# 0kam/alproj

Measured on AMD Instinct MI355X. Metric: Gpoints/s projected (pinhole + Brown-Conrady, single pose) over the 100M-vertex DSM; CMA-ES iterations/s in `cma`, higher is better.
Workload: dtype f32

## Files before the change

### alproj_amd/csrc/alp_raster.hip

```cpp
#include "alp_raster_internal.h"

#include <algorithm>
#include <atomic>
#include <climits>
#include <cmath>
#include <cstdlib>
#include <thread>
#include <type_traits>
#include <vector>

namespace alp {

#include "raster_dev.h"
#include "raster_common.h"
#include "raster_parked.h"
#include "raster_index.h"
#include "raster_plan.h"
#include "raster_grid.h"
#include "raster_large.h"
#include "raster_resolve.h"
#include "raster_post.h"

}

// ... 97 lines not shown
    for (auto &s : sums) {
        const unsigned here = s;
        s = (unsigned)run;
        run += here;
    }
    if ((long long)run != m->n_tri) return ALP_OK;
    e = hipMemcpyAsync(block_dev, sums.data(), (size_t)blocks * 4, hipMemcpyHostToDevice, st);
    if (e == hipSuccess) {
        hipLaunchKernelGGL(subgrid_rank_kernel, dim3((unsigned)blocks), dim3(256), 0, st, present, words, block_dev, rank);
        e = hipStreamSynchronize(st);
    }
    if (e != hipSuccess) return fail(ALP_EHIP, "sub-grid ranks: %s", hipGetErrorString(e));
    block_dev.reset();
    m->valid_derived = std::move(derived);
    if (int rc = apply_derived_mask(m, nullptr)) {
        reset_all(m->valid_derived, m->valid);
        return rc;
    }
    m->tri_present = std::move(present);
    m->tri_rank = std::move(rank);
    m->ind.reset();
    m->implicit = true;
    m->grid_h = gh;
    m->grid_w = gw;
    m->n_tri = full;
    return ALP_OK;
}

int ensure_gqueue(alp_mesh *m, unsigned cap) {
    if (m->gqueue && m->gcap >= cap) return ALP_OK;
    m->gcap = 0;
    if (int rc = m->gqueue.reserve((size_t)cap * sizeof(unsigned))) return rc;
    m->gcap = cap;
    return ALP_OK;
}

int finish_frame_of(alp_mesh *m);

int frame_valid_count(alp_mesh *m, int64_t *count) {
    if (int e = finish_frame_of(m)) return e;
    const long long npix = (long long)m->w * m->h;
    const int chunks = (int)((npix + COMPACT_CHUNK - 1) / COMPACT_CHUNK);
    if (chunks > m->compact_cap) {
        m->compact_cap = 0;
        reset_all(m->compact_counts, m->compact_offsets);
        const size_t counts = (size_t)chunks * (sizeof(unsigned) + 4 * sizeof(float)) + 16;
        const size_t offsets = (size_t)(chunks + 3) * sizeof(unsigned long long);
        if (int rc = reserve_all({counts, offsets}, m->compact_counts, m->compact_offsets)) return rc;
        m->compact_cap = chunks;
    }
    hipStream_t st = ctx().stream;
    ktime_begin();
    float *span = (float *)(((uintptr_t)(m->compact_counts + chunks) + 15) & ~(uintptr_t)15);
    hipLaunchKernelGGL(valid_count_kernel, dim3(chunks), dim3(256), 0, st, m->image, npix, m->compact_counts, span);
    hipLaunchKernelGGL(scan_counts_kernel, dim3(1), dim3(1024), 0, st, m->compact_counts, chunks, m->compact_offsets, span);
    ktime_end();
    ALP_HIP(hipGetLastError());
    unsigned long long tail[3] = {0, 0, 0};
    ALP_HIP(hipMemcpyAsync(tail, m->compact_offsets + chunks, sizeof(tail), hipMemcpyDeviceToHost, st));
    ALP_HIP(hipStreamSynchronize(st));
    const unsigned long long total = tail[0];
    memcpy(m->valid_span, tail + 1, sizeof(m->valid_span));
    m->valid_total = (int64_t)total;
    *count = m->valid_total;
    return ALP_OK;
}

int frame_valid_write(alp_mesh *m, const double *offsets, unsigned *idx_dev, double *xyz_dev, bool planar) {
    const long long npix = (long long)m->w * m->h;
    const int chunks = (int)((npix + COMPACT_CHUNK - 1) / COMPACT_CHUNK);
    const double o0 = offsets ? offsets[0] : 0.0, o1 = offsets ? offsets[1] : 0.0, o2 = offsets ? offsets[2] : 0.0;
    ktime_begin();
    hipLaunchKernelGGL(valid_write_kernel, dim3(chunks), dim3(256), 0, ctx().stream, m->image, npix, m->compact_offsets, o0, o1,
                       o2, idx_dev, xyz_dev, planar ? 1ll : 3ll, planar ? (long long)m->valid_total_planes : 1ll);
    ktime_end();
    ALP_HIP(hipGetLastError());
    return ALP_OK;
}

}

namespace {

int ensure_frame(alp_mesh *m, int w, int h) {
    if (m->w == w && m->h == h && m->vis) return ALP_OK;
    m->w = m->h = 0;
    m->vis_current = false;
    reset_all(m->vis, m->image);
    if (int rc = reserve_all({(size_t)w * h * sizeof(unsigned long long) + QC_TOTAL * sizeof(unsigned),
                              (size_t)w * h * 3 * sizeof(float)}, m->vis, m->image))
        return rc;
    m->hiz.reset();
    if (int rc = m->hiz.reserve((size_t)hiz_total(w, h) * sizeof(unsigned))) return rc;
    m->w = w;
    m->h = h;
    return ALP_OK;
}

unsigned *frame_counters(const alp_mesh *m, const View &v) { return (unsigned *)(m->vis + (size_t)v.w * v.h); }

host::FramePlan frame_plan_of(const alp_mesh *m, const View &v) {
    return host::frame_plan(m->implicit, m->grid_h, m->grid_w, m->n_tri, v.w, v.h, ctx().cu_count, GT_W, GT_H, RASTER_BLOCKS_PER_CU,
                            RESOLVE_BLOCKS_PER_CU);
}

template <bool IMPLICIT>
int drain_rare(alp_mesh *m, const View &v, const host::FramePlan &p, int round) {
    hipStream_t st = ctx().stream;
    unsigned *items = frame_counters(m, v) + QC_STRIDE * round, *general = items + 1;
    hipLaunchKernelGGL((raster_general_kernel<IMPLICIT>), dim3(p.general_wgs), dim3(256), 0, st, m->vert, m->ind,
                       (long long)m->grid_w, v, m->vis, m->gqueue, general, m->gcap, m->queue, items, m->qcap);
    ALP_HIP(hipGetLastError());
    hipLaunchKernelGGL((raster_large_kernel<IMPLICIT>), dim3(p.large_wgs), dim3(256), 0, st, m->vert, m->ind,
                       (long long)m->grid_w, v, m->vis, m->queue, items, m->qcap);
    ALP_HIP(hipGetLastError());
    return ALP_OK;
}

int drain_parked(alp_mesh *m, const View &v, const host::FramePlan &p, int round) {
    const unsigned *cap = round ? m->park_cap_b : m->park_cap;
    hipLaunchKernelGGL(raster_parked_kernel, dim3(p.parked_wgs[round]), dim3(256), 0, ctx().stream, v, m->vis,
                       m->park_small + (round ? m->park_cap[0] : 0), m->park_large + (round ? m->park_cap[1] : 0),
                       m->park_cell + (round ? m->park_cap[2] : 0), frame_counters(m, v) + QC_STRIDE * round + 2, cap[0], cap[1], cap[2]);
    ALP_HIP(hipGetLastError());
    return ALP_OK;
}

int ensure_grid_plan(alp_mesh *m, const host::FramePlan &p) {
    if (!m->park_small) {
        host::FrameQueues q;
        for (int k = 0; k < 3; ++k) q.park_b[k] = m->park_cap_b[k];
        host::initial_park_caps(initial_queue_cap(), &q);
        if (int e = alloc_park(m, q.park, q.park_b)) return e;
    }
    if (m->tile_bounds) return ALP_OK;
    DeviceBuffer<float> tb;
    DeviceBuffer<unsigned> tl;
    if (int rc = reserve_all({(size_t)p.tile_bounds_bytes, (size_t)p.tile_lists_bytes}, tb, tl)) return rc;
    hipLaunchKernelGGL(tile_bounds_kernel, dim3((unsigned)p.tiles), dim3(256), 0, ctx().stream, m->vert, (int)m->grid_h,
                       (int)m->grid_w, p.tiles_x, tb);
    const hipError_t e = hipGetLastError();
    if (e != hipSuccess) return fail(ALP_EHIP, "frame plan of the mesh: %s", hipGetErrorString(e));
    m->tile_bounds = std::move(tb);
    m->tile_lists = std::move(tl);
    return ALP_OK;
}

int grid_round(alp_mesh *m, const View &v, const host::FramePlan &p, int round, int along_rows, const unsigned *list,
               const unsigned *list_count, int patch_words) {
    unsigned *fcount = frame_counters(m, v);
    const unsigned *cap = round ? m->park_cap_b : m->park_cap;
    hipLaunchKernelGGL(raster_grid_kernel, dim3(p.grid_wgs), dim3(256), (size_t)patch_words * 8, ctx().stream, m->vert, m->valid,
                       (int)m->grid_h, (int)m->grid_w, v, m->vis, m->gqueue, fcount + 1, m->gcap, along_rows, list, list_count,
                       m->park_small + (round ? m->park_cap[0] : 0), m->park_large + (round ? m->park_cap[1] : 0),
                       m->park_cell + (round ? m->park_cap[2] : 0), fcount + QC_STRIDE * round + 2, cap[0], cap[1], cap[2], patch_words);
    ALP_HIP(hipGetLastError());
    return ALP_OK;
}

int draw_grid_mesh(alp_mesh *m, const View &v, const host::FramePlan &p) {
    hipStream_t st = ctx().stream;
    unsigned *near_list = m->tile_lists, *far_list = near_list + p.tiles, *second_list = far_list + p.tiles,
             *counts = frame_counters(m, v) + 2 * QC_STRIDE;
    TileCull cull;
    make_tile_cull(v, &cull);
    if (getenv("ALP_NO_TILE_CULL")) cull.enabled = 0;
    if (getenv("ALP_NO_OCCLUSION")) cull.occlusion = 0;
    int along_rows = std::fabs(v.R[0][2]) > std::fabs(v.R[0][0]);
    if (const char *e = dev_getenv("ALP_GRID_LANES")) along_rows = e[0] == 'r';
    hipLaunchKernelGGL(tile_plan_kernel, dim3(p.plan_grid), dim3(256), 0, st, m->tile_bounds, (unsigned)p.tiles, cull, near_list,
                       far_list, counts, counts + 4);
    ALP_HIP(hipGetLastError());
    static const int patch_near = patch_words_env("ALP_PATCH_NEAR", PATCH_WORDS_NEAR),
                     patch_far = patch_words_env("ALP_PATCH_FAR", PATCH_WORDS_FAR);
    if (int e = grid_round(m, v, p, 0, along_rows, near_list, counts + 0, patch_near)) return e;
    if (int e = dev_report_first_round(st, counts)) return e;
    const bool two_rounds = cull.enabled && cull.occlusion;
    if (!two_rounds)
        if (int e = drain_rare<true>(m, v, p, 0)) return e;
    if (int e = drain_parked(m, v, p, 0)) return e;
    if (two_rounds) {
        const HizDims dm = hiz_dims(v.w, v.h);
        hipLaunchKernelGGL(hiz_build_kernel, dim3((unsigned)dm.w[3], (unsigned)dm.h[3]), dim3(256), 0, st, m->vis, v.w, v.h, dm,
                           m->hiz, counts + 4);
        ALP_HIP(hipGetLastError());
        hipLaunchKernelGGL(tile_occlusion_kernel, dim3(p.plan_grid), dim3(256), 0, st, m->tile_bounds, cull, far_list, counts, dm,
                           m->hiz, second_list, counts + 2);
        ALP_HIP(hipGetLastError());
        if (int e = grid_round(m, v, p, 1, along_rows, second_list, counts + 2, patch_far)) return e;
        if (int e = drain_rare<true>(m, v, p, 0)) return e;
        if (int e = drain_parked(m, v, p, 1)) return e;
    }
    return dev_report_tiles(m, v, cull, p.tiles, p.plan_grid, two_rounds, counts);
}

int draw_indexed_mesh(alp_mesh *m, const View &v, const host::FramePlan &p) {
    hipLaunchKernelGGL((raster_kernel<false>), dim3(p.index_grid), dim3(256), 0, ctx().stream, m->vert, m->ind, m->valid,
                       (long long)m->n_tri, (long long)m->grid_w, v, m->vis, m->gqueue, frame_counters(m, v) + 1, m->gcap);
    ALP_HIP(hipGetLastError());
    return drain_rare<false>(m, v, p, 0);
}

template <bool IMPLICIT>
int resolve_frame(alp_mesh *m, const View &v, const RemapCoef &rc, double min_distance, const host::FramePlan &p) {
    const int identity = rc.a1 == 1 && rc.a2 == 1 && rc.k1 == 0 && rc.k2 == 0 && rc.k3 == 0 && rc.k4 == 0 && rc.k5 == 0 &&
                         rc.k6 == 0 && rc.p1 == 0 && rc.p2 == 0 && rc.s1 == 0 && rc.s2 == 0 && rc.s3 == 0 && rc.s4 == 0 &&
                         rc.c0 > 0 && rc.c1 > 0;
    hipLaunchKernelGGL((resolve_kernel<IMPLICIT>), dim3(p.resolve_grid), dim3(256), 0, ctx().stream, m->vert,
                       m->coords_as_value ? nullptr : m->value, m->ind, (long long)m->grid_w, v, rc, identity, min_distance, m->vis,
                       m->image, frame_counters(m, v), m->n_tri > 0 ? m->qcount_host : nullptr);
    ALP_HIP(hipGetLastError());
    return ALP_OK;
}

int render_impl(alp_mesh *m, const View &v, const RemapCoef &rc, double min_distance, bool resolve_only = false) {
    hipStream_t st = ctx().stream;
    const host::FramePlan p = frame_plan_of(m, v);
    m->vis_current = false;
    if (!resolve_only)
        ALP_HIP(hipMemsetAsync(m->vis, 0, (size_t)v.w * v.h * sizeof(unsigned long long) + QC_TOTAL * sizeof(unsigned), st));
    if (m->n_tri > 0 && !resolve_only) {
        if (m->implicit)
            if (int e = ensure_grid_plan(m, p)) return e;
        if (int e = m->implicit ? draw_grid_mesh(m, v, p) : draw_indexed_mesh(m, v, p)) return e;
    }
    if (int e = m->implicit ? resolve_frame<true>(m, v, rc, min_distance, p) : resolve_frame<false>(m, v, rc, min_distance, p)) return e;
    m->last_v = v;
    m->last_rc = rc;
    m->last_min_distance = min_distance;
    m->unchecked = m->n_tri > 0;
    m->vis_current = true;
    m->rz_n = -1;
    ++(resolve_only ? m->frames_resolve_only : m->frames_full);
    if (int e = dev_report_frame(st)) return e;
    m->rendered = true;
    return ALP_OK;
}

static bool same_view(const View &a, const View &b) {
    return a.w == b.w && a.h == b.h && a.fx == b.fx && a.fy == b.fy && a.sx == b.sx && a.sy == b.sy && a.fxd == b.fxd && a.fyd == b.fyd &&
           !memcmp(a.R, b.R, sizeof(a.R)) && !memcmp(a.camf, b.camf, sizeof(a.camf)) && !memcmp(a.caml, b.caml, sizeof(a.caml)) &&
           !memcmp(a.Rd, b.Rd, sizeof(a.Rd)) && !memcmp(a.camd, b.camd, sizeof(a.camd));
}

int finish_frame(alp_mesh *m) {
    while (m->unchecked) {
        ALP_HIP(hipStreamSynchronize(ctx().stream));
        m->unchecked = false;
        host::FrameQueues have;
        have.items = m->qcap;
        have.general = m->gcap;
        for (int k = 0; k < 3; ++k) {
            have.park[k] = m->park_cap[k];
            have.park_b[k] = m->park_cap_b[k];
        }
        const host::QueueVerdict want = host::frame_verdict(m->qcount_host, QC_STRIDE, m->park_small != nullptr, have);
        if (want.none()) break;
        if (want.park)
            if (int e = alloc_park(m, want.caps.park, want.caps.park_b)) return e;
        if (want.items)
            if (int e = ensure_queue(m, want.caps.items)) return e;
        if (want.general)
            if (int e = ensure_gqueue(m, want.caps.general)) return e;
        if (int e = render_impl(m, m->last_v, m->last_rc, m->last_min_distance)) return e;
    }
    return ALP_OK;
}

}

int alp::finish_frame_of(alp_mesh *m) { return finish_frame(m); }

int alp::upload_f32(float *dst, const void *src, int dtype, int64_t n_vert) {
    const size_t count = (size_t)n_vert * 3;
    if (dtype == ALP_F32) return upload_chunked(dst, src, count * 4);
    const size_t CH = (size_t)24 << 20;
    const size_t ch = count < CH ? count : CH;
    double *stage = nullptr;
    if (int rc = scratch_reserve(ch * 8, (void **)&stage)) return rc;
    hipStream_t st = ctx().stream;
    const hipError_t e = staged_upload(src, 8, (int64_t)count, (int64_t)ch, stage, [&](int64_t off, int64_t cnt) {
        hipLaunchKernelGGL(cast_f64_f32_kernel, dim3(4096), dim3(256), 0, st, stage, (long long)cnt, (long long)off, dst);
    });
    if (e != hipSuccess) return fail(ALP_EHIP, "float64 upload: %s", hipGetErrorString(e));
    ALP_HIP(hipStreamSynchronize(st));
    return ALP_OK;
}

static int streamed_grid_check(alp_mesh *m, const void *ind, int ind_dtype, int64_t n_tri, long long gw, bool *is_grid) {
    hipStream_t st = ctx().stream;
    const size_t esize = ind_dtype == ALP_I32 ? 4 : 8;
    const int64_t total = n_tri * 3;
    const int64_t CH = (int64_t)(((size_t)192 << 20) / esize) / 3 * 3;
    const int64_t ch = total < CH ? total : CH;
    void *stage = nullptr;
    if (int rc = scratch_reserve((size_t)ch * esize, &stage)) return rc;
    hipError_t e = hipMemsetAsync(m->qcount_dev, 0, sizeof(unsigned), st);
    if (e == hipSuccess)
        e = staged_upload(ind, esize, total, ch, stage, [&](int64_t off, int64_t cnt) {
            if (ind_dtype == ALP_I32)
                hipLaunchKernelGGL(check_grid_chunk_kernel<int>, dim3(4096), dim3(256), 0, st, (const int *)stage, cnt / 3, off / 3, gw, m->qcount_dev);
            else
                hipLaunchKernelGGL(check_grid_chunk_kernel<long long>, dim3(4096), dim3(256), 0, st, (const long long *)stage, cnt / 3, off / 3, gw,
// ... 123 lines not shown
int alp_mesh_destroy(alp_mesh_t *m) {
    if (!m) return ALP_OK;
    if (ctx().ready) hipStreamSynchronize(ctx().stream);
    delete m;
    return ALP_OK;
}

int alp_render_enqueue(alp_mesh_t *m, const double params[ALP_NPARAM], const double *offsets, double min_distance) {
    if (int rc = require_init()) return rc;
    ALP_REQUIRE(m && params, "NULL argument");
    ALP_REQUIRE(params[21] >= 1 && params[22] >= 1 && params[21] <= 32768 && params[22] <= 32768,
                "image size w,h must be in [1, 32768]");
    View v;
    RemapCoef rc;
    make_view(params, offsets, &v, &rc);
    if (int e = ensure_frame(m, v.w, v.h)) return e;
    const bool no_cache = getenv("ALP_NO_VIS_CACHE") != nullptr;
    const bool cached = m->vis_current && !no_cache && same_view(v, m->last_v);
    if (!m->ev_frame[0]) {
        Event a, b;
        if (int e = a.ensure()) return e;
        if (int e = b.ensure()) return e;
        m->ev_frame[0] = std::move(a);
        m->ev_frame[1] = std::move(b);
    }
    ALP_HIP(hipEventRecord(m->ev_frame[0], ctx().stream));
    const int e = render_impl(m, v, rc, min_distance, cached);
    if (e) return e;
    ALP_HIP(hipEventRecord(m->ev_frame[1], ctx().stream));
    return ALP_OK;
}

int alp_mesh_frame_ms(alp_mesh_t *m, float *ms) {
    if (int rc = require_init()) return rc;
    ALP_REQUIRE(m && ms, "NULL argument");
    if (!m->rendered || !m->ev_frame[1]) return fail(ALP_ESTATE, "alp_mesh_frame_ms: nothing rendered yet");
    ALP_HIP(hipEventSynchronize(m->ev_frame[1]));
    ALP_HIP(hipEventElapsedTime(ms, m->ev_frame[0], m->ev_frame[1]));
    return ALP_OK;
}

int alp_mesh_trim(alp_mesh_t *m) {
    if (int rc = require_init()) return rc;
    ALP_REQUIRE(m, "mesh handle is NULL");
    ALP_HIP(hipStreamSynchronize(ctx().stream));
    m->rz_work.reset();
    m->rz_points.reset();
    m->rz_n = -1;
    return ALP_OK;
}

int alp_render_fetch(alp_mesh_t *m, float *out) {
    if (int rc = require_init()) return rc;
    ALP_REQUIRE(m && out, "NULL argument");
    if (!m->rendered) return fail(ALP_ESTATE, "alp_render_fetch: nothing rendered yet");
    if (int e = finish_frame(m)) return e;
    ALP_HIP(hipMemcpyAsync(out, m->image, (size_t)m->w * m->h * 3 * sizeof(float), hipMemcpyDeviceToHost, ctx().stream));
    ALP_HIP(hipStreamSynchronize(ctx().stream));
    return ALP_OK;
}

int alp_render_fetch_u8(alp_mesh_t *m, float scale, int reverse_channels, uint8_t *out) {
    if (int rc = require_init()) return rc;
    ALP_REQUIRE(m && out, "NULL argument");
    if (!m->rendered) return fail(ALP_ESTATE, "alp_render_fetch_u8: nothing rendered yet");
    if (int e = finish_frame(m)) return e;
    const long long npix = (long long)m->w * m->h;
    unsigned char *dev = nullptr;
    if (int rc = scratch_reserve((size_t)npix * 3, (void **)&dev)) return rc;
    hipLaunchKernelGGL(image_u8_kernel, dim3(ctx().cu_count * 16), dim3(256), 0, ctx().stream, m->image, npix, scale,
                       reverse_channels, dev);
    ALP_HIP(hipGetLastError());
    ALP_HIP(hipMemcpyAsync(out, dev, (size_t)npix * 3, hipMemcpyDeviceToHost, ctx().stream));
    ALP_HIP(hipStreamSynchronize(ctx().stream));
    return ALP_OK;
}

int alp_render_fetch_visibility(alp_mesh_t *m, uint64_t *out) {
    if (int rc = require_init()) return rc;
    ALP_REQUIRE(m && out, "NULL argument");
    if (!m->rendered) return fail(ALP_ESTATE, "alp_render_fetch_visibility: nothing rendered yet");
    if (int e = finish_frame(m)) return e;
    const unsigned long long *src = m->vis;
    if (m->tri_present) {
        const long long npix = (long long)m->w * m->h;
        unsigned long long *tr = nullptr;
        if (int rc = scratch_reserve((size_t)npix * sizeof(uint64_t), (void **)&tr)) return rc;
        hipLaunchKernelGGL(vis_translate_kernel, dim3((unsigned)((npix + 255) / 256)), dim3(256), 0, ctx().stream, m->vis, npix,
                           m->tri_present, m->tri_rank, tr);
        ALP_HIP(hipGetLastError());
        src = tr;
    }
    ALP_HIP(hipMemcpyAsync(out, src, (size_t)m->w * m->h * sizeof(uint64_t), hipMemcpyDeviceToHost, ctx().stream));
    ALP_HIP(hipStreamSynchronize(ctx().stream));
    return ALP_OK;
}

int alp_render_gather(alp_mesh_t *m, const int32_t *u, const int32_t *v, int64_t n, const double *offsets,
                      double *xyz_out) {
    if (int rc = require_init()) return rc;
    ALP_REQUIRE(m, "mesh handle is NULL");
    ALP_REQUIRE(n >= 0, "n is negative");
    if (!m->rendered) return fail(ALP_ESTATE, "alp_render_gather: nothing rendered yet");
    if (int e = finish_frame(m)) return e;
    if (n == 0) return ALP_OK;
    ALP_REQUIRE(u && v && xyz_out, "NULL argument");
    char *dev = nullptr;
    const size_t uv_bytes = (size_t)n * sizeof(int32_t), xyz_bytes = (size_t)n * 3 * sizeof(double);
    if (int rc = scratch_reserve(xyz_bytes + 2 * uv_bytes, (void **)&dev)) return rc;
    double *xyz_dev = (double *)dev;
    int32_t *u_dev = (int32_t *)(dev + xyz_bytes), *v_dev = u_dev + n;
    hipStream_t st = ctx().stream;
    const double o0 = offsets ? offsets[0] : 0.0, o1 = offsets ? offsets[1] : 0.0, o2 = offsets ? offsets[2] : 0.0;
    hipError_t e = hipMemcpyAsync(u_dev, u, uv_bytes, hipMemcpyHostToDevice, st);
    if (e == hipSuccess) e = hipMemcpyAsync(v_dev, v, uv_bytes, hipMemcpyHostToDevice, st);
    if (e == hipSuccess) {
        KTimeScope kt;
        hipLaunchKernelGGL(gather_pixels_kernel, dim3((unsigned)((n + 255) / 256)), dim3(256), 0, st, m->image, m->w,
                           m->h, u_dev, v_dev, n, o0, o1, o2, xyz_dev);
        e = hipGetLastError();
    }
    if (e == hipSuccess) e = hipMemcpyAsync(xyz_out, xyz_dev, xyz_bytes, hipMemcpyDeviceToHost, st);
    if (e == hipSuccess) e = hipStreamSynchronize(st);
    if (e != hipSuccess) return fail(ALP_EHIP, "alp_render_gather: %s", hipGetErrorString(e));
    return ALP_OK;
}

int alp_distance_mask(const double *xyz, int64_t n, const double camera[3], double min_distance, double max_distance,
                      uint8_t *keep) {
    if (int rc = require_init()) return rc;
    ALP_REQUIRE(n >= 0, "n is negative");
    if (n == 0) return ALP_OK;
    ALP_REQUIRE(xyz && camera && keep, "NULL argument");
    ALP_REQUIRE(!(min_distance < 0), "min_distance must be non-negative");
    ALP_REQUIRE(!(max_distance < min_distance), "max_distance must be >= min_distance");
    char *dev = nullptr;
    const size_t xyz_bytes = (size_t)n * 3 * sizeof(double);
    if (int rc = scratch_reserve(xyz_bytes + (size_t)n, (void **)&dev)) return rc;
    unsigned char *keep_dev = (unsigned char *)(dev + xyz_bytes);
    hipStream_t st = ctx().stream;
    hipError_t e = hipMemcpyAsync(dev, xyz, xyz_bytes, hipMemcpyHostToDevice, st);
    if (e == hipSuccess) {
        KTimeScope kt;
        hipLaunchKernelGGL(distance_mask_kernel, dim3((unsigned)((n + 255) / 256)), dim3(256), 0, st, (const double *)dev,
                           (long long)n, camera[0], camera[1], camera[2], min_distance, max_distance, keep_dev);
        e = hipGetLastError();
    }
    if (e == hipSuccess) e = hipMemcpyAsync(keep, keep_dev, (size_t)n, hipMemcpyDeviceToHost, st);
    if (e == hipSuccess) e = hipStreamSynchronize(st);
    if (e != hipSuccess) return fail(ALP_EHIP, "alp_distance_mask: %s", hipGetErrorString(e));
    return ALP_OK;
}

int alp_render_valid_count(alp_mesh_t *m, int64_t *count) {
    if (int rc = require_init()) return rc;
    ALP_REQUIRE(m && count, "NULL argument");
    if (!m->rendered) return fail(ALP_ESTATE, "alp_render_valid_count: nothing rendered yet");
    return frame_valid_count(m, count);
}

static int take_valid_total(alp_mesh_t *m, const char *who, int64_t *M) {
    if (int rc = require_init()) return rc;
    if (!m) return fail(ALP_EINVAL, "%s: mesh handle is NULL", who);
    if (m->valid_total < 0) return fail(ALP_ESTATE, "%s: call alp_render_valid_count first", who);
    *M = m->valid_total;
    m->valid_total = -1;
    return ALP_OK;
}

int alp_render_fetch_valid(alp_mesh_t *m, const double *offsets, uint32_t *idx_out, double *xyz_out) {
    int64_t M = 0;
// ... 66 lines not shown
    {
        KTimeScope kt;
        const dim3 grid((unsigned)((M + 255) / 256));
#define ALP_COLUMNS(A) hipLaunchKernelGGL(table_columns_kernel<A>, grid, dim3(256), 0, st, idx_dev, (long long)M, m->w, (const A *)arr_dev, \
                                          (int)channels, index_dev, u_dev, v_dev, block_dev + 3 * M)
        if (array_dtype == ALP_U8) ALP_COLUMNS(unsigned char);
        else if (array_dtype == ALP_U16) ALP_COLUMNS(unsigned short);
        else if (array_dtype == ALP_F32) ALP_COLUMNS(float);
        else ALP_COLUMNS(double);
#undef ALP_COLUMNS
    }
    hipError_t e = hipGetLastError();
    if (e == hipSuccess) e = hipMemcpyAsync(block_out, block_dev, block_bytes, hipMemcpyDeviceToHost, st);
    if (e == hipSuccess) e = hipMemcpyAsync(index_out, index_dev, (size_t)M * 8, hipMemcpyDeviceToHost, st);
    if (e == hipSuccess) e = hipMemcpyAsync(u_out, u_dev, (size_t)M * 2, hipMemcpyDeviceToHost, st);
    if (e == hipSuccess) e = hipMemcpyAsync(v_out, v_dev, (size_t)M * 2, hipMemcpyDeviceToHost, st);
    if (e == hipSuccess) e = hipStreamSynchronize(st);
    if (e != hipSuccess) return fail(ALP_EHIP, "alp_render_fetch_valid_table: %s", hipGetErrorString(e));
    return ALP_OK;
}

int alp_render(alp_mesh_t *m, const double params[ALP_NPARAM], const double *offsets, double min_distance, float *out) {
    if (int rc = alp_render_enqueue(m, params, offsets, min_distance)) return rc;
    return alp_render_fetch(m, out);
}

static void distort_setup(int64_t h, int64_t w, const double coeffs[14], RemapCoef *rc, int *grid) {
    double p[ALP_NPARAM] = {0};
    for (int i = 0; i < 14; ++i) p[7 + i] = coeffs[i];
    p[3] = 60; p[21] = (double)w; p[22] = (double)h;
    View v;
    make_view(p, nullptr, &v, rc);
    const long long want = ((long long)h * w + 255) / 256;
    *grid = (int)(want < 4096 ? want : 4096);
}

int alp_distort_image(const float *img, int64_t h, int64_t w, int64_t c, const double coeffs[14], float *out) {
    if (int rc = require_init()) return rc;
    ALP_REQUIRE(img && out && coeffs, "NULL argument");
    ALP_REQUIRE(h >= 1 && w >= 1 && c >= 1 && h <= 32768 && w <= 32768, "bad image shape");
    RemapCoef rc;
    int grid = 0;
    distort_setup(h, w, coeffs, &rc, &grid);
    const size_t bytes = (size_t)h * w * c * sizeof(float);
    float *dev = nullptr;
    if (int e2 = scratch_reserve(2 * bytes, (void **)&dev)) return e2;
    hipError_t e = hipMemcpyAsync(dev, img, bytes, hipMemcpyHostToDevice, ctx().stream);
    if (e == hipSuccess) {
        hipLaunchKernelGGL(distort_image_kernel, dim3(grid), dim3(256), 0, ctx().stream, dev, (int)w, (int)h, (int)c, rc,
                           (float *)((char *)dev + bytes));
        e = hipMemcpyAsync(out, (char *)dev + bytes, bytes, hipMemcpyDeviceToHost, ctx().stream);
    }
    if (e == hipSuccess) e = hipStreamSynchronize(ctx().stream);
    if (e != hipSuccess) return fail(ALP_EHIP, "alp_distort_image: %s", hipGetErrorString(e));
    return ALP_OK;
}

int alp_distort_map(int64_t h, int64_t w, const double coeffs[14], float *map_x, float *map_y) {
    if (int rc = require_init()) return rc;
    ALP_REQUIRE(coeffs && map_x && map_y, "NULL argument");
    ALP_REQUIRE(h >= 1 && w >= 1 && h <= 32768 && w <= 32768, "bad image shape");
    RemapCoef rc;
    int grid = 0;
    distort_setup(h, w, coeffs, &rc, &grid);
    const size_t bytes = (size_t)h * w * sizeof(float);
    float *dev = nullptr;
    if (int e2 = scratch_reserve(2 * bytes, (void **)&dev)) return e2;
    hipLaunchKernelGGL(distort_map_kernel, dim3(grid), dim3(256), 0, ctx().stream, (int)w, (int)h, rc, dev, dev + (size_t)h * w);
    ALP_HIP(hipGetLastError());
    ALP_HIP(hipMemcpyAsync(map_x, dev, bytes, hipMemcpyDeviceToHost, ctx().stream));
    ALP_HIP(hipMemcpyAsync(map_y, dev + (size_t)h * w, bytes, hipMemcpyDeviceToHost, ctx().stream));
    ALP_HIP(hipStreamSynchronize(ctx().stream));
    return ALP_OK;
}

int alp_render_load(alp_mesh_t *m, const float *image, int64_t h, int64_t w) {
    if (int rc = require_init()) return rc;
    ALP_REQUIRE(m && image, "NULL argument");
    ALP_REQUIRE(h >= 1 && w >= 1 && h <= 32768 && w <= 32768, "image size w,h must be in [1, 32768]");
    if (m->unchecked) ALP_HIP(hipStreamSynchronize(ctx().stream));
    m->unchecked = false;
    if (int e = ensure_frame(m, (int)w, (int)h)) return e;
    if (int e = upload_chunked(m->image, image, (size_t)h * w * 3 * sizeof(float))) return e;
    ALP_HIP(hipMemsetAsync(m->vis, 0, (size_t)h * w * sizeof(unsigned long long), ctx().stream));
    m->vis_current = false;
    m->rz_n = -1;
    m->rendered = true;
    m->valid_total = -1;
    return ALP_OK;
}

}
```

### alproj_amd/csrc/alp_raster_internal.h

```cpp
#pragma once
#include "alp_internal.h"

namespace alp {

struct View {
    float R[3][3];
    float camf[3], caml[3];
    float fx, fy, sx, sy;
    int w, h;
    double fxd, fyd;
    double kx, ky, ifx, ify;
    double Rd[3][3], camd[3];
};

struct RemapCoef {
    double a1, a2, k1, k2, k3, k4, k5, k6, p1, p2, s1, s2, s3, s4, c0, c1;
};

struct WorkItem { unsigned tri; unsigned short sub, tx, ty, pad; };

struct Deferred {
    int X[3], Y[3];
    float iw[3];
    unsigned t;
};

struct alignas(16) ParkedCell {
    int X[4], Y[4];
    float iw[4];
    unsigned cell;
    unsigned pad[3];
};

}

struct alp_mesh {
    int64_t n_vert = 0, n_tri = 0, grid_h = 0, grid_w = 0;
    bool implicit = false;
    alp::DeviceBuffer<float> vert, value;
    alp::DeviceBuffer<int> ind;
    alp::DeviceBuffer<unsigned char> valid;
    alp::DeviceBuffer<unsigned char> valid_derived;
    alp::DeviceBuffer<unsigned> tri_present;
    alp::DeviceBuffer<unsigned> tri_rank;
    alp::DeviceBuffer<float> tile_bounds;
    alp::DeviceBuffer<unsigned> tile_lists;
    alp::DeviceBuffer<unsigned> hiz;
    bool coords_as_value = false;
    int w = 0, h = 0;
    alp::DeviceBuffer<unsigned long long> vis;
    alp::DeviceBuffer<float> image;
    alp::DeviceBuffer<alp::WorkItem> queue;
    unsigned qcap = 0;
    alp::DeviceBuffer<unsigned> gqueue;
    unsigned gcap = 0;
    alp::DeviceBuffer<alp::Deferred> park_small;
    alp::Deferred *park_large = nullptr;
    alp::DeviceBuffer<alp::ParkedCell> park_cell;
    unsigned park_cap[3] = {0, 0, 0};
    unsigned park_cap_b[3] = {0, 0, 0};
    alp::DeviceBuffer<unsigned> qcount_dev;
    alp::PinnedBuffer<unsigned> qcount_host;
    bool unchecked = false;
    alp::View last_v;
    alp::RemapCoef last_rc;
    double last_min_distance = 0;
    bool rendered = false;
    bool vis_current = false;
    int64_t frames_full = 0, frames_resolve_only = 0;
    alp::DeviceBuffer<unsigned> compact_counts;
    alp::DeviceBuffer<unsigned long long> compact_offsets;
    int compact_cap = 0;
    float valid_span[4] = {0, 0, 0, 0};
    int64_t valid_total = -1;
    int64_t valid_total_planes = 0;
    alp::DeviceBuffer<char> rz_points;
    int64_t rz_n = -1;
    alp::DeviceBuffer<char> rz_work;
    alp::Event ev_frame[2];
};

namespace alp {
int upload_chunked(void *dst, const void *src, size_t bytes);
int upload_f32(float *dst, const void *src, int dtype, int64_t n_vert);
int ensure_queue(alp_mesh *m, unsigned cap);
int ensure_gqueue(alp_mesh *m, unsigned cap);
constexpr int QC_STRIDE = 8;
constexpr int QC_TOTAL = 2 * QC_STRIDE + 8;
unsigned initial_queue_cap();
int frame_valid_count(alp_mesh *m, int64_t *count);
int frame_valid_write(alp_mesh *m, const double *offsets, unsigned *idx_dev, double *xyz_dev, bool planar);
int apply_derived_mask(alp_mesh *m, const unsigned char *user);
// ... 2 lines not shown
```

### alproj_amd/csrc/host/alp_host_selfcheck.cpp

```cpp
#include <cinttypes>
#include <mutex>
#include <random>
#include <string>
#include <utility>

#include "host/alp_host.h"
#include "host/alp_buffer.h"

using namespace alp;

namespace {

std::atomic<int> g_failures{0};
std::mutex g_print;

#define CHECK(cond, ...)                                           \
    do {                                                           \
        if (!(cond)) {                                             \
            std::lock_guard<std::mutex> lk(g_print);               \
            fprintf(stderr, "CHECK FAILED %s:%d: %s | ", __FILE__, __LINE__, #cond); \
            fprintf(stderr, __VA_ARGS__);                          \
            fprintf(stderr, "\n");                                 \
            g_failures.fetch_add(1);                               \
        }                                                          \
// ... 366 lines not shown
                    const int64_t blocks = ((int64_t)f[0] * f[1] + 255) / 256;
                    CHECK(p.resolve_grid >= 1 && p.resolve_grid <= 64 * cu && p.resolve_grid == std::min<int64_t>(blocks, 64 * cu),
                          "resolve grid %d for %d x %d at %d CUs", p.resolve_grid, f[0], f[1], cu);
                }
            }
    for (int cu : {1, 64, 256, 304})
        for (int64_t n_tri : {(int64_t)1, (int64_t)255, (int64_t)256, (int64_t)257, (int64_t)64 * 256 * cu - 1, (int64_t)64 * 256 * cu,
                              (int64_t)64 * 256 * cu + 1, (int64_t)199960002, ((int64_t)1 << 32) - 2}) {
            const host::FramePlan p = host::frame_plan(false, 0, 0, n_tri, 1, 1, cu, TW, TH);
            CHECK(p.index_grid >= 1 && p.index_grid <= 64 * cu && p.index_grid == std::min<int64_t>((n_tri + 255) / 256, 64 * cu) && p.tiles == 0 &&
                      p.grid_wgs == 0 && p.resolve_grid == 1, "index grid %d for %" PRId64 " triangles at %d CUs", p.index_grid, n_tri, cu);
            const host::FramePlan q = host::frame_plan(false, 0, 0, n_tri, 5616, 3744, cu, TW, TH, 16, 8);
            CHECK(q.index_grid == std::min<int64_t>((n_tri + 255) / 256, 16 * cu) && q.resolve_grid == std::min<int64_t>(82134, 8 * cu), "tunable caps");
        }
    CHECK(host::initial_queue_cap(nullptr) == (1u << 20) && host::initial_queue_cap("8") == 8 && host::initial_queue_cap("0") == (1u << 20) &&
              host::initial_queue_cap("-3") == (1u << 20) && host::initial_queue_cap("1073741824") == (1u << 20) &&
              host::initial_queue_cap("1073741823") == 1073741823u && host::initial_queue_cap("x") == (1u << 20), "ALP_QUEUE_CAP");
    for (unsigned cap : {1u, 8u, 1000u, 1u << 20, (1u << 20) + 1, (1u << 30) - 1}) {
        host::FrameQueues q;
        host::initial_park_caps(cap, &q);
        CHECK(q.park[0] == cap && q.park[1] == cap && q.park[2] == (cap == (1u << 20) ? 2u << 20 : cap), "parked queues of a start at %u", cap);
        for (int k = 0; k < 3; ++k) CHECK(q.park_b[k] == q.park[k] / 8 + 64, "second round of a start at %u", cap);
    }
    std::mt19937_64 rng(6);
    const unsigned levels[] = {0, 1, 7, 8, 9, 72, 1000, 1u << 20, (1u << 20) + 1, 3000000, 1u << 31};
    auto pick = [&] { return levels[rng() % (sizeof(levels) / sizeof(levels[0]))]; };
    for (int trial = 0; trial < 20000; ++trial) {
        const int stride = 8;
        unsigned c[16];
        for (unsigned &x : c) x = pick();
        host::FrameQueues have;
        have.items = std::max(pick(), 1u);
        have.general = std::max(pick(), 1u);
        const bool has_park = trial % 4 != 0;
        if (has_park) {
            host::FrameQueues start;
            host::initial_park_caps(std::max(pick(), 1u), &start);
            for (int k = 0; k < 3; ++k) {
                have.park[k] = trial % 3 ? start.park[k] : std::max(pick(), 1u);
                have.park_b[k] = trial % 3 ? start.park_b[k] : std::max(pick(), 1u);
            }
        }
        const host::QueueVerdict v = host::frame_verdict(c, stride, has_park, have);
        const unsigned items = std::max(c[0], c[stride]), general = std::max(c[1], c[stride + 1]);
        CHECK(v.items == (items > have.items) && v.general == (general > have.general), "work items / general entries: which overflowed");
        CHECK(v.items ? v.caps.items > items : v.caps.items == have.items, "work items %u of %u -> %u", items, have.items, v.caps.items);
        CHECK(v.general ? v.caps.general > general : v.caps.general == have.general, "general entries %u of %u -> %u", general, have.general, v.caps.general);
        bool park_over = false;
        for (int k = 0; k < 3; ++k) {
            const unsigned a = c[2 + k], b = c[stride + 2 + k];
            park_over |= has_park && (a > have.park[k] || b > have.park_b[k]);
            if (!has_park) {
                CHECK(v.caps.park[k] == have.park[k] && v.caps.park_b[k] == have.park_b[k], "parked counters count although no parked queues exist");
                continue;
            }
            CHECK(a > have.park[k] ? v.caps.park[k] > a : v.caps.park[k] == have.park[k], "first round, kind %d: %u of %u -> %u", k, a, have.park[k],
                  v.caps.park[k]);
            CHECK(v.caps.park_b[k] >= have.park_b[k] && v.caps.park_b[k] >= b, "second round, kind %d: %u of %u -> %u", k, b, have.park_b[k], v.caps.park_b[k]);
            CHECK(!v.park || v.caps.park_b[k] >= v.caps.park[k] / 8 + 64, "second round, kind %d, below an eighth of the first", k);
        }
        CHECK(v.park == park_over, "parked queues: which overflowed");
        if (!v.park)
            for (int k = 0; k < 3; ++k) CHECK(v.caps.park_b[k] == have.park_b[k], "second round changed without an overflow");
        CHECK(v.none() == !(v.items || v.general || v.park), "none()");
        const host::QueueVerdict again = host::frame_verdict(c, stride, has_park, v.caps);
        CHECK(again.none(), "the verdict on the grown queues is not none");
        CHECK(again.caps.items == v.caps.items && again.caps.general == v.caps.general, "none changes a capacity");
        for (int k = 0; k < 3; ++k) CHECK(again.caps.park[k] == v.caps.park[k] && again.caps.park_b[k] == v.caps.park_b[k], "none changes a capacity");
    }
}

void check_row_div() {
    for (uint32_t w = 2; w <= 65536; ++w) {
        const RowDiv rd = host::row_div(w);
        const uint64_t mul = (((uint64_t)1 << rd.shift) + w - 1) / w;
        if (rd.w != w || mul > 0xffffffffull || rd.mul != (uint32_t)mul) CHECK(false, "row_div(%u): mul does not fit 32 bits", w);
        const uint32_t top = 0x7fffffffu, kmax = top / w;
        bool ok = true;
        for (uint32_t e : {0u, 1u, w - 1, w, w + 1, top, top - w + 1, kmax * w, kmax * w - 1}) ok &= rd.div(e) == e / w;
        for (uint32_t k = 1; k <= kmax; k += 1 + k / 3 + (w & 7)) {
            ok &= rd.div(k * w) == k && rd.div(k * w - 1) == k - 1;
        }
        if (!ok) CHECK(false, "RowDiv::div is not e / %u somewhere below 2^31", w);
    }
}

template <int VEC>
uint32_t row_walk_vector(const RowDiv &rd, uint32_t e0, uint32_t last) {
    const uint32_t w = rd.w;
    const RowWalk<VEC> walk(rd, e0, last);
    bool ok = walk.one_row == (e0 % w + VEC <= w);
    for (uint32_t k = 0; k < (uint32_t)VEC; ++k) {
        uint32_t col = ~0u, row0 = ~0u;
        walk.at(k, &col, &row0);
        const uint32_t e = std::min(e0 + k, last);
        if (e0 + k <= last || !walk.one_row) ok &= col == e % w && row0 == e / w * w;
        else ok &= col == e0 % w + k && row0 == e0 / w * w;
        ok &= col < w && row0 <= last;
    }
    if (!ok) CHECK(false, "RowWalk<%d>: w=%u e0=%u last=%u", VEC, w, e0, last);
    return walk.one_row ? 0 : 1;
}

template <int VEC>
void check_row_walk_t() {
    for (uint32_t w = 1; w <= 64; ++w) {
        const RowDiv rd = host::row_div(w);
        for (uint32_t n = w + 1; n <= 4 * w + VEC + 1; ++n) {
            uint32_t crossing = 0;
            for (uint32_t e0 = 0; e0 < n; e0 += VEC) crossing += row_walk_vector<VEC>(rd, e0, n - 1);
            if (w % VEC == 0) CHECK(crossing == 0, "RowWalk<%d>: w=%u n=%u leaves the one-row form", VEC, w, n);
        }
    }
    std::mt19937_64 rng(VEC);
    for (int t = 0; t < 4000; ++t) {
        const uint32_t w = t < 8 ? 65536 - t : 1 + (uint32_t)(rng() % 65536);
        const RowDiv rd = host::row_div(w);
        const uint32_t n = 0x80000000u - (uint32_t)(rng() % (2 * w + 8));
        const uint32_t last = n - 1, rows = last / w;
        for (uint32_t r = rows >= 3 ? rows - 3 : 0; r <= rows; ++r)
            for (uint32_t e0 = (r * w - std::min(r * w, (uint32_t)(2 * VEC))) / VEC * VEC; e0 <= last && e0 < r * w + 2 * VEC; e0 += VEC)
                row_walk_vector<VEC>(rd, e0, last);
        for (uint32_t e0 = (last - std::min(last, (uint32_t)(3 * VEC))) / VEC * VEC; e0 <= last; e0 += VEC) row_walk_vector<VEC>(rd, e0, last);
        for (int s = 0; s < 16; ++s) row_walk_vector<VEC>(rd, (uint32_t)(rng() % n) / VEC * VEC, last);
    }
}

void check_row_walk() {
    check_row_walk_t<2>();
    check_row_walk_t<4>();
}

void check_match_plan() {
    for (int len = 1; len <= MATCH_MAX_LEN; ++len) {
        const int ks = host::match_ksteps(len);
        int want = 0;
        for (int c = 1; c <= 16 && !want; ++c) {
            bool listed = false;
            for (int k : MATCH_KSTEPS) listed = listed || k == c;
            if (listed && c * MATCH_K >= len) want = c;
        }
        CHECK(ks == want && ks * MATCH_K >= len, "match_ksteps(%d) = %d, not %d", len, ks, want);
    }
    CHECK(host::match_ksteps(61) == 2 && host::match_ksteps(128) == 4 && host::match_ksteps(MATCH_MAX_LEN) == 16, "AKAZE / SIFT / longest");
    const int64_t edges[] = {0, 1, 2, 3, 31, 32, 33, 63, 64, 65, 127, 128, 129, 255, 256, 257, 511, 512, 513, 4096, 50000, 1000003};
    const int lens[] = {1, 31, 32, 33, 61, 64, 65, 96, 97, 128, 129, 192, 193, 256, 257, 384, 385, 512};
    for (int len : lens)
        for (int esize : {1, 4})
            for (int cu : {1, 64, 256})
                for (int64_t nq : edges)
                    for (int64_t nt : edges) {
                        if (nt < 2) continue;
                        const int64_t tiles = (nt + 31) / 32;
                        for (int forced : {0, 1, 2, 3, (int)std::min<int64_t>(tiles, 1 << 20)}) {
                            const host::MatchPlan p = host::match_plan(nq, nt, len, esize, forced, cu);
                            CHECK(p.padded_len == p.ksteps * 32 && p.padded_len >= len && p.groups == (p.ksteps <= 4 ? 2 : 1) &&
                                      p.query_tile == 128 * p.groups && p.train_tile == 32,
                                  "tiles of len %d", len);
                            CHECK(p.train_tiles == tiles && p.nt_pad == tiles * 32 && p.nt_pad >= nt && p.nt_pad - nt < 32, "train tiles of %" PRId64, nt);
                            CHECK(p.nq_pad % p.query_tile == 0 && p.nq_pad >= nq && p.nq_pad - nq < p.query_tile && p.query_tiles * p.query_tile == p.nq_pad,
                                  "query tiles of %" PRId64, nq);
                            if (forced > tiles) continue;
                            if (forced) CHECK(p.splits == forced, "forced splits %d -> %d", forced, p.splits);
                            else {
                                int64_t s = 1;
                                while (s < tiles && s * p.query_tiles < 2 * cu) ++s;
// ... 422 lines not shown
    using Mem = CountedMemory;
    using Bytes = Buffer<Mem, unsigned char>;
    {
        Bytes b;
        CHECK(!b && b.get() == nullptr && b.capacity() == 0 && Mem::live == 0, "a new buffer is not empty");
        CHECK(b.reserve(100) == ALP_OK && b && b.capacity() == 100 && Mem::live == 1, "first reserve");
        unsigned char *first = b;
        b[99] = 7;
        CHECK(b.reserve(100) == ALP_OK && b.reserve(1) == ALP_OK && b.get() == first && b.capacity() == 100 && b[99] == 7,
              "a reserve that fits moved the block");
        CHECK(Mem::live == 1, "a reserve that fits left %d blocks", Mem::live);
        Mem::peak = Mem::live;
        CHECK(b.reserve(101) == ALP_OK && b.capacity() == 101 && Mem::live == 1 && Mem::peak == 1,
              "growing held %d blocks at once", Mem::peak);
        b[100] = 1;
        Mem::fail_next(1);
        CHECK(b.reserve(1000) == ALP_EHIP && !b && b.capacity() == 0 && Mem::live == 0,
              "a failed reserve left %d block(s)", Mem::live);
        CHECK(strstr(alp_last_error(), "counted allocation") != nullptr, "error text: %s", alp_last_error());
        Mem::fail_next(0);
        CHECK(b.reserve(8) == ALP_OK && b.capacity() == 8 && Mem::live == 1, "reserve after a failure");
        b.reset();
        CHECK(!b && b.capacity() == 0 && Mem::live == 0, "reset");
        b.reset();
        CHECK(Mem::live == 0, "second reset");
    }
    {
        Bytes a;
        CHECK(a.reserve(16) == ALP_OK, "reserve");
        unsigned char *pa = a;
        Bytes b(std::move(a));
        CHECK(!a && a.capacity() == 0 && b.get() == pa && b.capacity() == 16 && Mem::live == 1, "move construction");
        Bytes c;
        c = std::move(b);
        CHECK(!b && c.get() == pa && c.capacity() == 16 && Mem::live == 1, "move assignment to an empty buffer");
        Bytes d;
        CHECK(d.reserve(32) == ALP_OK && Mem::live == 2, "reserve");
        d = std::move(c);
        CHECK(!c && d.get() == pa && d.capacity() == 16 && Mem::live == 1, "move assignment onto a block left %d live", Mem::live);
        Bytes &self = d;
        d = std::move(self);
        CHECK(d.get() == pa && Mem::live == 1, "self-assignment");
        Buffer<Mem> v;
        CHECK(v.reserve(8) == ALP_OK && (const float *)v == (const float *)v.get() && (char *)v + 4 == (char *)v.get() + 4, "casts");
    }
    CHECK(Mem::live == 0, "%d block(s) outlived their buffers", Mem::live);
    for (int size = 2; size <= 3; ++size)
        for (int bad = 1; bad <= size; ++bad)
            for (int held = 0; held < 2; ++held) {
                Buffer<Mem, double> x;
                Buffer<Mem> y;
                Buffer<Mem, int> z;
                auto group = [&](size_t n) {
                    return size == 2 ? reserve_all({n, 2 * n}, x, y) : reserve_all({n, 2 * n, 3 * n}, x, y, z);
                };
                if (held) CHECK(group(8) == ALP_OK && Mem::live == size, "first group");
                Mem::fail_next(bad);
                CHECK(group(64) == ALP_EHIP && !x && !y && !z && x.capacity() + y.capacity() + z.capacity() == 0 && Mem::live == 0,
                      "group of %d, member %d failed (held %d): %d block(s) live", size, bad, held, Mem::live);
                Mem::fail_next(0);
                CHECK(group(64) == ALP_OK && x && y && (size == 2 || z) && x.capacity() == 64 && y.capacity() == 128,
                      "group of %d after a failure", size);
                CHECK(Mem::live == size, "group of %d after a failure: %d blocks", size, Mem::live);
                x[7] = 1.0;
                ((char *)y)[127] = 1;
                if (size == 3) z[47] = 1;
                double *px = x;
                CHECK(group(64) == ALP_OK && x.get() == px && Mem::live == size, "a group that fits moved");
                reset_all(x, y, z);
                CHECK(Mem::live == 0, "reset_all");
            }
    CHECK(Mem::live == 0, "%d block(s) live at the end", Mem::live);
}

int main(int argc, char **argv) {
    if (argc > 2 && !strcmp(argv[1], "--canary")) return canary(argv[2]);
    if (argc > 1 && !strcmp(argv[1], "--plan")) return plan(argc - 2, argv + 2);
    if (argc > 1 && !strcmp(argv[1], "--lm")) return lm_mode();
    struct Group { const char *name; void (*fn)(); };
    const Group groups[] = {{"hash", check_hash},     {"minmax", check_minmax},   {"prefault", check_prefault}, {"fold_pose", check_fold_pose},
                            {"convert", check_convert}, {"grid", check_grid},     {"selection", check_selection}, {"errors", check_errors},
                            {"plan", check_plan},       {"frame_plan", check_frame_plan}, {"row_div", check_row_div}, {"lm", check_lm},
                            {"buffer", check_buffer},   {"row_walk", check_row_walk}, {"match_plan", check_match_plan},
                            {"epi_plan", check_epi_plan}};
    const bool concurrent = !(argc > 1 && !strcmp(argv[1], "--serial"));
    std::vector<std::thread> th;
    for (const Group &g : groups) {
        if (concurrent) th.emplace_back(g.fn);
        else g.fn();
    }
    for (auto &x : th) x.join();
    std::thread a(check_convert), b(check_convert);
    check_selection();
    a.join();
    b.join();
    if (g_failures.load()) {
        fprintf(stderr, "host selfcheck: %d comparison(s) failed\n", g_failures.load());
        return 1;
    }
    printf("host selfcheck ok: %zu groups%s\n", sizeof(groups) / sizeof(groups[0]), concurrent ? ", run concurrently" : "");
    return 0;
}
```

### alproj_amd/csrc/host/alp_plan.h

```cpp
#pragma once

#include <cstdint>
#include <cstdlib>

namespace alp {

struct RowDiv {
    uint32_t w = 0, shift = 0, mul = 0;
    ALP_HD uint32_t div(uint32_t e) const { return (uint32_t)(((uint64_t)e * mul) >> shift); }
};

template <int VEC>
struct RowWalk {
    RowDiv rd;
    uint32_t c, r0, room;
    bool one_row;
    ALP_HD RowWalk(const RowDiv &d, uint32_t e0, uint32_t last) : rd(d) {
        const uint32_t r = d.div(e0);
        r0 = r * d.w;
        c = e0 - r0;
        room = last - e0;
        one_row = d.w % VEC == 0 || c + VEC <= d.w;
    }
    ALP_HD void at(uint32_t k, uint32_t *col, uint32_t *row0) const {
        if (one_row) {
            *col = c + k;
            *row0 = r0;
        } else if (rd.w >= VEC) {
            const uint32_t ck = c + (k < room ? k : room);
            const bool next = ck >= rd.w;
            *col = next ? ck - rd.w : ck;
            *row0 = next ? r0 + rd.w : r0;
        } else {
            const uint32_t e = r0 + c + (k < room ? k : room), r = rd.div(e);
            *col = e - r * rd.w;
            *row0 = r * rd.w;
        }
    }
};

namespace host {

inline RowDiv row_div(uint32_t w) {
    RowDiv rd;
    uint32_t l = 0;
    while ((1u << l) < w) ++l;
    rd.w = w;
    rd.shift = 31 + l;
    rd.mul = (uint32_t)((((uint64_t)1 << rd.shift) + w - 1) / w);
    return rd;
}

inline int stream_grid(int64_t items, int cu_count) {
    const int64_t want = (items + 255) / 256;
    const int64_t cap = (int64_t)cu_count * 8;
    return (int)(want < 1 ? 1 : (want < cap ? want : cap));
}

constexpr int64_t RES_CHUNK_BYTES = (int64_t)256 << 20;
inline int64_t stage_chunk_points(int64_t n, int64_t pairs_per_point) {
    int64_t chunk = RES_CHUNK_BYTES / (pairs_per_point * 16) / 1024 * 1024;
    if (chunk < 1024) chunk = 1024;
    return chunk > n ? n : chunk;
}

inline int confirm_grid(int64_t n, int cu_count) {
    const int64_t rows = (n + 255) / 256, want = (int64_t)cu_count * 4;
    return (int)(rows < want ? (rows > 0 ? rows : 1) : want);
}

constexpr int64_t POP_BATCHED_PARTIALS_BYTES = (int64_t)128 << 20;

struct PopGrid { int stripes, tile_cols; };

inline PopGrid pop_grid(int64_t n, int64_t P, bool is_f64, int V, int TC, int cu_count, bool batched, int ov_stripes = 0,
                        int ov_tile_cols = 0) {
    int nblk = cu_count * (is_f64 ? 24 : 4), ytiles = 1;
    const int64_t rows = (n + 255) / 256, tiles = (P + TC - 1) / TC;
    if (!is_f64) {
        const int64_t want = (rows + 4 * V - 1) / (4 * V);
        const int64_t lo = (int64_t)cu_count * 4, hi = (int64_t)cu_count * 64;
        const int64_t rounded = (want + lo - 1) / lo * lo;
        nblk = (int)(want < lo ? lo : (want > hi ? hi : (want < 4 * lo ? rounded : want)));
        if (tiles >= 2) {
            int64_t k = (int64_t)((double)rows / ((double)V * 2.12 * (double)lo) + 0.5);
            k = k < 1 ? 1 : (k > 16 ? 16 : k);
            const int64_t stripes = (rows + V * k - 1) / (V * k);
            if (stripes * tiles >= 4 * lo) { nblk = (int)stripes; ytiles = (int)tiles; }
        }
    } else {
        const int64_t cap = ((int64_t)128 << 20) / (8 * P);
        const int64_t lo = (int64_t)cu_count * 3;
        if (nblk > cap) nblk = (int)(cap > lo ? cap : lo);
    }
    if (ov_stripes >= 1 && ov_tile_cols >= 1 && ov_tile_cols <= tiles) { nblk = ov_stripes; ytiles = ov_tile_cols; }
    if (rows < nblk) nblk = (int)(rows > 0 ? rows : 1);
    if (batched) {
        const int64_t cap = POP_BATCHED_PARTIALS_BYTES / (8 * P);
        if (nblk > cap) nblk = (int)(cap > 1 ? cap : 1);
        const int64_t fill = (int64_t)cu_count * 4;
        if (ytiles == 1 && tiles >= 2 && nblk < fill) {
            const int64_t cols = (fill + nblk - 1) / nblk;
            ytiles = (int)(cols < tiles ? cols : tiles);
        }
    }
    return {nblk, ytiles};
}

inline PopGrid mend_grid(int64_t n, int64_t P, int V, int TC, int cu_count) {
    const int64_t rows = (n + 255) / 256, tiles = (P + TC - 1) / TC;
    const int64_t lo = (int64_t)cu_count * 3, hi = (int64_t)cu_count * 24;
    int64_t nblk = (rows + 4 * V - 1) / (4 * V);
    nblk = nblk < lo ? lo : (nblk > hi ? hi : nblk);
    const int64_t cap = POP_BATCHED_PARTIALS_BYTES / (8 * (P > 0 ? P : 1));
    if (nblk > cap) nblk = cap;
    if (nblk > rows) nblk = rows;
    if (nblk < 1) nblk = 1;
    return {(int)nblk, (int)(tiles > 0 ? tiles : 1)};
}

// ... 106 lines not shown
```

### alproj_amd/csrc/raster_common.h

```cpp
#pragma once

constexpr int SUB = 256;
constexpr float COORD_LIMIT = 4194304.0f;
constexpr int SMALL_PIXELS = 32;
constexpr int TILE = 64;

static void make_view(const double *p, const double *offsets, View *v, RemapCoef *rc) {
    double x = p[0], y = p[1], z = p[2];
    if (offsets) { x -= offsets[0]; y -= offsets[2]; z -= offsets[1]; }
    const double pi = M_PI;
    const double pan = (360 - p[4]) * pi / 180, tilt = p[5] * pi / 180, roll = p[6] * pi / 180;
    const double rx[3][3] = {{1, 0, 0}, {0, std::cos(tilt), -std::sin(tilt)}, {0, std::sin(tilt), std::cos(tilt)}};
    const double ry[3][3] = {{std::cos(pan), 0, std::sin(pan)}, {0, 1, 0}, {-std::sin(pan), 0, std::cos(pan)}};
    const double rz[3][3] = {{std::cos(roll), -std::sin(roll), 0}, {std::sin(roll), std::cos(roll), 0}, {0, 0, 1}};
    double t[3][3];
    for (int i = 0; i < 3; ++i)
        for (int j = 0; j < 3; ++j) {
            double s = 0;
            for (int k = 0; k < 3; ++k) s += rz[i][k] * rx[k][j];
            t[i][j] = s;
        }
    for (int i = 0; i < 3; ++i)
        for (int j = 0; j < 3; ++j) {
            double s = 0;
            for (int k = 0; k < 3; ++k) s += t[i][k] * ry[k][j];
            v->R[i][j] = (float)s;
            v->Rd[i][j] = s;
        }
    const double cam[3] = {x, z, y};
    for (int i = 0; i < 3; ++i) {
        v->camd[i] = cam[i];
        v->camf[i] = (float)cam[i];
        v->caml[i] = (float)(cam[i] - (double)v->camf[i]);
    }
    const double w = p[21], h = p[22];
    const double fov_x = p[3] * pi / 180, fov_y = fov_x * h / w;
    v->fxd = 1 / std::tan(fov_x / 2);
    v->fyd = 1 / std::tan(fov_y / 2);
    v->fx = (float)v->fxd;
    v->fy = (float)v->fyd;
    v->w = (int)w;
    v->h = (int)h;
    v->sx = 0.5f * (float)v->w;
    v->sy = 0.5f * (float)v->h;
    v->kx = 1.0 / (double)v->sx;
    v->ky = 1.0 / (double)v->sy;
    v->ifx = 1.0 / v->fxd;
    v->ify = 1.0 / v->fyd;
    if (rc) {
        rc->a1 = 1 / p[7]; rc->a2 = 1 / p[8];
        rc->k1 = -p[9]; rc->k2 = -p[10]; rc->k3 = -p[11]; rc->k4 = -p[12]; rc->k5 = -p[13]; rc->k6 = -p[14];
        rc->p1 = -p[15]; rc->p2 = -p[16]; rc->s1 = -p[17]; rc->s2 = -p[18]; rc->s3 = -p[19]; rc->s4 = -p[20];
        rc->c0 = (double)(float)((w - 1) / 2.0);
        rc->c1 = (double)(float)((h - 1) / 2.0);
    }
}

#ifdef ALP_WG_TIMING
__device__ unsigned long long g_wgtime[8 * 131072];
#define WGT(k) do { if (threadIdx.x == 0 && blockIdx.x < 131072) g_wgtime[8 * blockIdx.x + (k)] = __builtin_amdgcn_s_memrealtime(); } while (0)
#else
#define WGT(k) ((void)0)
#endif
#ifdef ALP_RASTER_STATS
__device__ unsigned long long g_rstat[24 + 8 * 8];

#define RSTAT(k, n) atomicAdd(&g_rstat[k], (unsigned long long)(n))
#else
#define RSTAT(k, n) ((void)0)
#endif
__device__ __forceinline__ void to_view(const View &v, float px, float py, float pz, float out[3]) {
    const float dx = (px - v.camf[0]) - v.caml[0];
    const float dy = (py - v.camf[1]) - v.caml[1];
    const float dz = (pz - v.camf[2]) - v.caml[2];
#pragma unroll
    for (int i = 0; i < 3; ++i)
        out[i] = __builtin_fmaf(v.R[i][0], dx, __builtin_fmaf(v.R[i][1], dy, v.R[i][2] * dz));
}

__device__ __forceinline__ float exact_rcp_unchecked(float x) {
#if defined(__gfx950__)
    const float y = __builtin_amdgcn_rcpf(x);
    return __builtin_fmaf(y, __builtin_fmaf(-x, y, 1.0f), y);
#else
    return 1.0f / x;
#endif
}
__device__ __forceinline__ float exact_rcp(float x) {
    if (__builtin_expect(!(x >= 1.0f && x < 1.0e18f), 0)) return 1.0f / x;
    return exact_rcp_unchecked(x);
}

__device__ __forceinline__ void to_window(const View &v, const float q[3], float &xw, float &yw, float &iw) {
    const float i = exact_rcp(q[2]);
    iw = i;
    xw = __builtin_fmaf((v.fx * q[0]) * i, v.sx, v.sx);
    yw = __builtin_fmaf((v.fy * q[1]) * i, v.sy, v.sy);
}

__device__ __forceinline__ long long floor_div(long long a, long long b) {
    long long q = a / b;
    return (a % b != 0 && ((a < 0) != (b < 0))) ? q - 1 : q;
}

struct Idx3 { long long a, b, c; };

template <bool IMPLICIT>
__device__ __forceinline__ Idx3 tri_vertices(const int *__restrict__ ind, long long gw, long long t) {
    Idx3 r;
    if constexpr (IMPLICIT) {
        const unsigned cell = (unsigned)t >> 1, gc = (unsigned)gw - 1u, row = cell / gc, col = cell - row * gc;
        const long long a = (long long)(row * (unsigned)gw + col);
        r.a = a;
        r.b = (t & 1) ? a + gw + 1 : a + gw;
        r.c = (t & 1) ? a + 1 : a + gw + 1;
    } else {
        r.a = ind[t * 3 + 0];
        r.b = ind[t * 3 + 1];
        r.c = ind[t * 3 + 2];
    }
    return r;
}

struct TriSetup {
    long long X[3], Y[3];
    long long area2;
    int i0, i1, j0, j1;
    float iw[3];
    bool valid;
};

__device__ __forceinline__ int snap(float w) { return (int)__builtin_rintf(w * (float)SUB); }

__device__ __forceinline__ TriSetup setup_snapped(const View &v, const int X[3], const int Y[3],
                                                  const float iw[3]) {
    TriSetup s;
    s.valid = false;
#pragma unroll
    for (int k = 0; k < 3; ++k) {
        s.X[k] = X[k];
        s.Y[k] = Y[k];
        s.iw[k] = iw[k];
    }
    s.area2 = (s.X[1] - s.X[0]) * (s.Y[2] - s.Y[0]) - (s.X[2] - s.X[0]) * (s.Y[1] - s.Y[0]);
    if (s.area2 <= 0) return s;
    long long minx = s.X[0], maxx = s.X[0], miny = s.Y[0], maxy = s.Y[0];
#pragma unroll
    for (int k = 1; k < 3; ++k) {
        minx = s.X[k] < minx ? s.X[k] : minx;
        maxx = s.X[k] > maxx ? s.X[k] : maxx;
        miny = s.Y[k] < miny ? s.Y[k] : miny;
        maxy = s.Y[k] > maxy ? s.Y[k] : maxy;
    }
    long long i0 = -floor_div(-(minx - SUB / 2), SUB), i1 = floor_div(maxx - SUB / 2, SUB);
    long long j0 = -floor_div(-(miny - SUB / 2), SUB), j1 = floor_div(maxy - SUB / 2, SUB);
    if (i0 < 0) i0 = 0;
    if (j0 < 0) j0 = 0;
    if (i1 > v.w - 1) i1 = v.w - 1;
    if (j1 > v.h - 1) j1 = v.h - 1;
    if (i0 > i1 || j0 > j1) return s;
    s.i0 = (int)i0; s.i1 = (int)i1; s.j0 = (int)j0; s.j1 = (int)j1;
    s.valid = true;
    return s;
}

__device__ __forceinline__ TriSetup setup_tri(const View &v, const float xw[3], const float yw[3],
                                              const float iw[3]) {
    const int X[3] = {snap(xw[0]), snap(xw[1]), snap(xw[2])};
    const int Y[3] = {snap(yw[0]), snap(yw[1]), snap(yw[2])};
    return setup_snapped(v, X, Y, iw);
}

__device__ __forceinline__ unsigned long long pixel_key(const TriSetup &s, int i, int j, unsigned tri) {
    const long long px = (long long)i * SUB + SUB / 2, py = (long long)j * SUB + SUB / 2;
    long long e[3];
#pragma unroll
    for (int k = 0; k < 3; ++k) {
        const int a = (k + 1) % 3, b = (k + 2) % 3;
        const long long dx = s.X[b] - s.X[a], dy = s.Y[b] - s.Y[a];
        e[k] = dx * (py - s.Y[a]) - dy * (px - s.X[a]);
        if (e[k] < 0 || (e[k] == 0 && !(dy < 0 || (dy == 0 && dx > 0)))) return 0ull;
    }
    const float q = __builtin_fmaf((float)e[2], s.iw[2], __builtin_fmaf((float)e[1], s.iw[1], (float)e[0] * s.iw[0])) *
                    (1.0f / (float)s.area2);
    return ((unsigned long long)__float_as_uint(q) << 32) | (unsigned long long)(0xFFFFFFFFu - tri);
}

__device__ __forceinline__ void vis_max(unsigned long long *vis, const View &v, int i, int j, unsigned long long key) {
    unsigned long long *dst = vis + (unsigned)(__umul24((unsigned)j, (unsigned)v.w) + (unsigned)i);
#ifdef VIS_PLAIN_STORE
    __builtin_nontemporal_store(key, dst);
#elif defined(VIS_NEVER)
    if (key == 0x123456789ull) atomicMax(dst, key);
#else
    atomicMax(dst, key);
#endif
}

__device__ __forceinline__ void raster_bbox(const TriSetup &s, unsigned tri, unsigned long long *vis, const View &v) {
    long long dx[3], dy[3], row[3];
    bool tl[3];
    const long long px0 = (long long)s.i0 * SUB + SUB / 2, py0 = (long long)s.j0 * SUB + SUB / 2;
#pragma unroll
    for (int k = 0; k < 3; ++k) {
        const int a = (k + 1) % 3, b = (k + 2) % 3;
        dx[k] = s.X[b] - s.X[a];
        dy[k] = s.Y[b] - s.Y[a];
        row[k] = dx[k] * (py0 - s.Y[a]) - dy[k] * (px0 - s.X[a]);
        tl[k] = dy[k] < 0 || (dy[k] == 0 && dx[k] > 0);
    }
    const float inv_area = 1.0f / (float)s.area2;
    for (int j = s.j0; j <= s.j1; ++j) {
        long long e0 = row[0], e1 = row[1], e2 = row[2];
        for (int i = s.i0; i <= s.i1; ++i) {
            const bool in0 = e0 > 0 || (e0 == 0 && tl[0]);
            const bool in1 = e1 > 0 || (e1 == 0 && tl[1]);
            const bool in2 = e2 > 0 || (e2 == 0 && tl[2]);
            if (in0 && in1 && in2) {
                const float q = __builtin_fmaf((float)e2, s.iw[2], __builtin_fmaf((float)e1, s.iw[1], (float)e0 * s.iw[0])) *
                                inv_area;
                vis_max(vis, v, i, j, ((unsigned long long)__float_as_uint(q) << 32) | (unsigned long long)(0xFFFFFFFFu - tri));
            }
            e0 -= dy[0] * SUB;
            e1 -= dy[1] * SUB;
            e2 -= dy[2] * SUB;
        }
        row[0] += dx[0] * SUB;
        row[1] += dx[1] * SUB;
        row[2] += dx[2] * SUB;
    }
}

__device__ void raster_big(const View &v, const float q[3][3], unsigned tri, unsigned long long *vis, int lane) {
    double xh[3], yh[3], wh[3];
    for (int k = 0; k < 3; ++k) {
        wh[k] = q[k][2];
        xh[k] = ((double)v.fx * q[k][0] + wh[k]) * v.sx;
        yh[k] = ((double)v.fy * q[k][1] + wh[k]) * v.sy;
    }
    const double det = xh[0] * (yh[1] * wh[2] - yh[2] * wh[1]) - yh[0] * (xh[1] * wh[2] - xh[2] * wh[1]) +
                       wh[0] * (xh[1] * yh[2] - xh[2] * yh[1]);
    if (!(det > 0)) return;
    const long long npix = (long long)v.w * v.h;
    for (long long p = lane; p < npix; p += 64) {
        {
            const int j = (int)(p / v.w), i = (int)(p - (long long)j * v.w);
            const double px = i + 0.5, py = j + 0.5;
            double e[3];
            bool inside = true;
            for (int k = 0; k < 3; ++k) {
                const int a = (k + 1) % 3, b = (k + 2) % 3;
                e[k] = px * (yh[a] * wh[b] - yh[b] * wh[a]) - py * (xh[a] * wh[b] - xh[b] * wh[a]) +
                       (xh[a] * yh[b] - xh[b] * yh[a]);
                if (!(e[k] > 0)) inside = false;
            }
            if (!inside) continue;
            const float qq = (float)((e[0] + e[1] + e[2]) / det);
            if (!(qq <= 1.0f)) continue;
            vis_max(vis, v, i, j, ((unsigned long long)__float_as_uint(qq) << 32) | (unsigned long long)(0xFFFFFFFFu - tri));
        }
    }
}


__device__ __forceinline__ int clip_project(const View &v, const float q[3][3], float xw[4], float yw[4],
                                            float iw[4], bool &big) {
    const bool in0 = q[0][2] >= 1.0f, in1 = q[1][2] >= 1.0f, in2 = q[2][2] >= 1.0f;
    const int nin = (int)in0 + (int)in1 + (int)in2;
    big = false;
    if (nin == 0) return 0;
    {
        bool r = true, l = true, t = true, b = true;
#pragma unroll
        for (int k = 0; k < 3; ++k) {
            const float cx = v.fx * q[k][0], cy = v.fy * q[k][1], cw = q[k][2];
            r = r && cx > cw;
            l = l && cx < -cw;
            t = t && cy > cw;
            b = b && cy < -cw;
        }
        if (r || l || t || b) return 0;
    }
    int np = 0;
    if (nin == 3) {
#pragma unroll
        for (int k = 0; k < 3; ++k) to_window(v, q[k], xw[k], yw[k], iw[k]);
        np = 3;
    } else {
        float poly[4][3];
        const bool in[3] = {in0, in1, in2};
#pragma unroll
        for (int k = 0; k < 3; ++k) {
            const int n = (k + 1) % 3;
            if (in[k]) { poly[np][0] = q[k][0]; poly[np][1] = q[k][1]; poly[np][2] = q[k][2]; ++np; }
            if (in[k] != in[n]) {
                const float *pi_ = in[k] ? q[k] : q[n];
                const float *po = in[k] ? q[n] : q[k];
                const float t = (1.0f - pi_[2]) / (po[2] - pi_[2]);
                poly[np][0] = __builtin_fmaf(t, po[0] - pi_[0], pi_[0]);
                poly[np][1] = __builtin_fmaf(t, po[1] - pi_[1], pi_[1]);
                poly[np][2] = 1.0f;
                ++np;
            }
        }
        for (int k = 0; k < np; ++k) to_window(v, poly[k], xw[k], yw[k], iw[k]);
    }
    for (int k = 0; k < np; ++k)
        if (!(fabsf(xw[k]) < COORD_LIMIT) || !(fabsf(yw[k]) < COORD_LIMIT)) big = true;
    return np - 2;
}

template <bool IMPLICIT>
__device__ __forceinline__ void load_view_tri(const View &v, const float *__restrict__ vert,
                                              const int *__restrict__ ind, long long gw, long long t,
                                              float q[3][3]) {
    const Idx3 id = tri_vertices<IMPLICIT>(ind, gw, t);
    const long long ids[3] = {id.a, id.b, id.c};
#pragma unroll
    for (int k = 0; k < 3; ++k) {
        const float *p = vert + 3 * ids[k];
        to_view(v, p[0], p[1], p[2], q[k]);
    }
}

#ifndef INLINE_LOG2
#define INLINE_LOG2 14
#endif
__device__ __forceinline__ int mul24(int a, int b) { return __mul24(a, b); }

#ifndef FAST_MAX
#define FAST_MAX 4
#endif
#ifndef COOP_MIN_W
#define COOP_MIN_W 3
#endif
#ifndef COOP_MIN_PIX
#define COOP_MIN_PIX 9
#endif


__device__ __forceinline__ void coop_raster(const View &v, const int X[3], const int Y[3], const float iw3[3],
                                            unsigned t, unsigned long long *__restrict__ vis, int lane) {
    const int minx = min(X[0], min(X[1], X[2])), maxx = max(X[0], max(X[1], X[2]));
    const int miny = min(Y[0], min(Y[1], Y[2])), maxy = max(Y[0], max(Y[1], Y[2]));
    const int ci0 = max((minx + SUB / 2 - 1) >> 8, 0), ci1 = min((maxx - SUB / 2) >> 8, v.w - 1);
    const int cj0 = max((miny + SUB / 2 - 1) >> 8, 0), cj1 = min((maxy - SUB / 2) >> 8, v.h - 1);
    const int area2 = (X[1] - X[0]) * (Y[2] - Y[0]) - (X[2] - X[0]) * (Y[1] - Y[0]);
    int dx[3], dy[3], bias[3], xa[3], ya[3];
#pragma unroll
    for (int k = 0; k < 3; ++k) {
        const int a = (k + 1) % 3, b = (k + 2) % 3;
        dx[k] = X[b] - X[a];
        dy[k] = Y[b] - Y[a];
        xa[k] = X[a];
        ya[k] = Y[a];
        bias[k] = (dy[k] < 0 || (dy[k] == 0 && dx[k] > 0)) ? 0 : 1;
    }
    const float inv_area = exact_rcp_unchecked((float)area2);
    const unsigned long long lo = (unsigned long long)(0xFFFFFFFFu - t);
    const int lx = lane & 7, ly = lane >> 3;
    for (int by = cj0; by <= cj1; by += 8)
        for (int bx = ci0 & ~7; bx <= ci1; bx += 8) {
            const int i = bx + lx, j = by + ly;
            if (i < ci0 || i > ci1 || j > cj1) continue;
            const int px = i * SUB + SUB / 2, py = j * SUB + SUB / 2;
            const int w0 = mul24(dx[0], py - ya[0]) - mul24(dy[0], px - xa[0]) - bias[0];
            const int w1 = mul24(dx[1], py - ya[1]) - mul24(dy[1], px - xa[1]) - bias[1];
            const int w2 = mul24(dx[2], py - ya[2]) - mul24(dy[2], px - xa[2]) - bias[2];
            if ((w0 | w1 | w2) >= 0) {
                RSTAT(7, 1);
                const float q = __builtin_fmaf((float)(w2 + bias[2]), iw3[2],
                                               __builtin_fmaf((float)(w1 + bias[1]), iw3[1],
                                                              (float)(w0 + bias[0]) * iw3[0])) * inv_area;
                vis_max(vis, v, i, j, ((unsigned long long)__float_as_uint(q) << 32) | lo);
            }
        }
}

__device__ __forceinline__ void coop_drain(const View &v, bool parked, const Deferred &d,
                                           unsigned long long *__restrict__ vis) {
    unsigned long long mask = __ballot(parked);
    const int lane = (int)(threadIdx.x & 63);
    while (mask) {
        const int src = __ffsll((long long)mask) - 1;
        mask &= mask - 1;
        int X[3], Y[3];
        float iw3[3];
#pragma unroll
        for (int k = 0; k < 3; ++k) {
            X[k] = __builtin_amdgcn_readlane(d.X[k], src);
            Y[k] = __builtin_amdgcn_readlane(d.Y[k], src);
            iw3[k] = __int_as_float(__builtin_amdgcn_readlane(__float_as_int(d.iw[k]), src));
        }
        const unsigned t = (unsigned)__builtin_amdgcn_readlane((int)d.t, src);
        if (lane == 0) RSTAT(8, 1);
        coop_raster(v, X, Y, iw3, t, vis, lane);
    }
}

enum { EMIT_DONE = 0, EMIT_PARKED = 1, EMIT_GENERAL = 2, EMIT_PARKED_SMALL = 3 };

__device__ __forceinline__ int emit_small(const View &v, const int X[3], const int Y[3], const float *iwsrc,
                                          int n0, int n1, int n2, unsigned t, unsigned long long *__restrict__ vis,
                                          Deferred *park, bool may_park, int coop_min_w = COOP_MIN_W,
                                          int coop_min_pix = COOP_MIN_PIX, bool tell_small = false) {
    const int minx = min(X[0], min(X[1], X[2])), maxx = max(X[0], max(X[1], X[2]));
    const int miny = min(Y[0], min(Y[1], Y[2])), maxy = max(Y[0], max(Y[1], Y[2]));
    const int i0 = (minx + SUB / 2 - 1) >> 8, i1 = (maxx - SUB / 2) >> 8;
    const int j0 = (miny + SUB / 2 - 1) >> 8, j1 = (maxy - SUB / 2) >> 8;
    if (i0 > i1 || j0 > j1 || i1 < 0 || j1 < 0 || i0 > v.w - 1 || j0 > v.h - 1) return EMIT_DONE;
    if (!(maxx - minx < (1 << INLINE_LOG2) && maxy - miny < (1 << INLINE_LOG2))) return EMIT_GENERAL;
    const int area2 = mul24(X[1] - X[0], Y[2] - Y[0]) - mul24(X[2] - X[0], Y[1] - Y[0]);
    if (area2 <= 0) return EMIT_DONE;
    const int ci0 = max(i0, 0), ci1 = min(i1, v.w - 1), cj0 = max(j0, 0), cj1 = min(j1, v.h - 1);
    const float iw3[3] = {iwsrc[n0], iwsrc[n1], iwsrc[n2]};
    if (may_park && ci1 - ci0 + 1 >= coop_min_w && mul24(ci1 - ci0 + 1, cj1 - cj0 + 1) >= coop_min_pix) {
#pragma unroll
        for (int k = 0; k < 3; ++k) {
            park->X[k] = X[k];
            park->Y[k] = Y[k];
            park->iw[k] = iw3[k];
        }
        park->t = t;
        return (tell_small && ci1 - ci0 < 8 && cj1 - cj0 < 8) ? EMIT_PARKED_SMALL : EMIT_PARKED;
    }
    const int px0 = ci0 * SUB + SUB / 2, py0 = cj0 * SUB + SUB / 2;
    int dx[3], dy[3], row[3], bias[3];
#pragma unroll
    for (int k = 0; k < 3; ++k) {
        const int a = (k + 1) % 3, b = (k + 2) % 3;
        dx[k] = X[b] - X[a];
        dy[k] = Y[b] - Y[a];
        bias[k] = (dy[k] < 0 || (dy[k] == 0 && dx[k] > 0)) ? 0 : 1;
        row[k] = mul24(dx[k], py0 - Y[a]) - mul24(dy[k], px0 - X[a]) - bias[k];
    }
    const float inv_area = exact_rcp_unchecked((float)area2);
    const unsigned long long lo = (unsigned long long)(0xFFFFFFFFu - t);
    RSTAT(2, 1);
    for (int j = cj0; j <= cj1; ++j) {
        int w0 = row[0], w1 = row[1], w2 = row[2];
        for (int i = ci0; i <= ci1; ++i) {
            if ((w0 | w1 | w2) >= 0) {
                RSTAT((ci1 - ci0) == 0 ? 3 : (ci1 - ci0) < 3 ? 4 : (ci1 - ci0) < 7 ? 5 : 6, 1);
                const float q = __builtin_fmaf((float)(w2 + bias[2]), iw3[2],
                                               __builtin_fmaf((float)(w1 + bias[1]), iw3[1],
                                                              (float)(w0 + bias[0]) * iw3[0])) * inv_area;
                vis_max(vis, v, i, j, ((unsigned long long)__float_as_uint(q) << 32) | lo);
// ... 52 lines not shown
```

### alproj_amd/csrc/raster_dev.h

```cpp
#pragma once

#if defined(ALP_WG_TIMING) || defined(ALP_RASTER_STATS) || defined(VIS_PLAIN_STORE) || defined(VIS_NEVER) || defined(PARK_NOATOMIC) || \
    defined(PARKED_SKIP_CELLS) || defined(PARKED_SKIP_COOP) || defined(PARKED_SKIP_COOP4) || defined(GRID_STOP_AFTER) ||               \
    defined(GRID_NO_XCD_SWIZZLE)
#define ALP_DEV_SWITCHES 1
#ifndef ALP_DEV
#error "development switch given without -DALP_DEV: this would build a library that renders wrong images"
#endif
#endif
#if defined(INLINE_LOG2) || defined(FAST_MAX) || defined(COOP_MIN_W) || defined(COOP_MIN_PIX) || defined(GT_W_LOG2) || defined(GT_H_LOG2) || \
    defined(HIZ_SPAN) || defined(GRID_WAVES_PER_EU) || defined(PATCH_MIN_FAST) || defined(PATCH_WORDS_NEAR) || defined(PATCH_WORDS_FAR) ||    \
    defined(RASTER_BLOCKS_PER_CU) || defined(RESOLVE_BLOCKS_PER_CU)
#define ALP_DEV_TUNABLES 1
#ifndef ALP_DEV
#error "tuning parameter overridden without -DALP_DEV"
#endif
#endif

const char *raster_dev_flags() {
    return ""
#ifdef ALP_DEV
           "ALP_DEV,"
#endif
#ifdef ALP_DEV_TUNABLES
           "tunables-overridden,"
#endif
#ifdef ALP_WG_TIMING
           "ALP_WG_TIMING,"
#endif
#ifdef ALP_RASTER_STATS
           "ALP_RASTER_STATS,"
#endif
#ifdef VIS_PLAIN_STORE
           "VIS_PLAIN_STORE(wrong image),"
#endif
#ifdef VIS_NEVER
           "VIS_NEVER(wrong image),"
#endif
#ifdef PARK_NOATOMIC
           "PARK_NOATOMIC(wrong image),"
#endif
#if defined(PARKED_SKIP_CELLS) || defined(PARKED_SKIP_COOP) || defined(PARKED_SKIP_COOP4)
           "PARKED_SKIP_*(wrong image),"
#endif
#ifdef GRID_STOP_AFTER
           "GRID_STOP_AFTER(wrong image),"
#endif
#ifdef GRID_NO_XCD_SWIZZLE
           "GRID_NO_XCD_SWIZZLE,"
#endif
        ;
}

#ifdef ALP_DEV
static const char *dev_getenv(const char *name) { return getenv(name); }
#else
static const char *dev_getenv(const char *) { return nullptr; }
#endif

static int patch_words_env(const char *name, int dflt) {
    if (const char *e = dev_getenv(name)) {
        const long w = atol(e);
        if (w >= 0 && w <= 5632) return (int)w;
    }
    return dflt;
}

struct TileCull;

#if defined(ALP_WG_TIMING) || defined(ALP_RASTER_STATS)
#include "raster_common.h"
#include "raster_parked.h"
#include "raster_index.h"
#include "raster_plan.h"
#endif

#ifdef ALP_WG_TIMING
static int dev_report_first_round(hipStream_t st, const unsigned *counts) {
    ALP_HIP(hipStreamSynchronize(st));
    unsigned hc[4];
    ALP_HIP(hipMemcpy(hc, counts, sizeof(hc), hipMemcpyDeviceToHost));
    std::vector<unsigned long long> tt(8 * (size_t)hc[0]);
    ALP_HIP(hipMemcpyFromSymbol(tt.data(), HIP_SYMBOL(g_wgtime), tt.size() * 8));
    unsigned long long t0 = ~0ull, t1 = 0;
    std::vector<double> dur;
    double phase[4] = {0, 0, 0, 0};
    for (unsigned i = 0; i < hc[0] && i < 131072; ++i) {
        t0 = std::min(t0, tt[8 * i]);
        t1 = std::max(t1, tt[8 * i + 4]);
        dur.push_back((tt[8 * i + 4] - tt[8 * i]) / 100.0);
        for (int k = 0; k < 4; ++k) phase[k] += (tt[8 * i + k + 1] - tt[8 * i + k]) / 100.0;
    }
    std::vector<double> sorted = dur;
    std::sort(sorted.begin(), sorted.end());
    double sum = 0;
// ... 67 lines not shown
```

### alproj_amd/csrc/raster_grid.h

```cpp
#pragma once

#ifndef GRID_WAVES_PER_EU
#define GRID_WAVES_PER_EU 8
#endif
#ifndef PATCH_MIN_FAST
#define PATCH_MIN_FAST 64
#endif
#ifndef PATCH_WORDS_NEAR
#define PATCH_WORDS_NEAR 4096
#endif
#ifndef PATCH_WORDS_FAR
#define PATCH_WORDS_FAR 0
#endif
__global__ __launch_bounds__(256) __attribute__((amdgpu_waves_per_eu(GRID_WAVES_PER_EU)))
void raster_grid_kernel(const float *__restrict__ vert, const unsigned char *__restrict__ valid, int gh, int gw, View v,
                        unsigned long long *__restrict__ vis, unsigned *__restrict__ gqueue,
                        unsigned *__restrict__ gcount, unsigned gcap, int lanes_along_rows,
                        const unsigned *__restrict__ tile_list, const unsigned *__restrict__ tile_count,
                        Deferred *__restrict__ park_small, Deferred *__restrict__ park_large,
                        ParkedCell *__restrict__ park_cell, unsigned *__restrict__ park_counts, unsigned park_cap_small,
                        unsigned park_cap_large, unsigned park_cap_cell, int patch_cap) {
    constexpr int BEHIND = INT_MIN, RANGE = INT_MIN + 1, NODATA = INT_MIN + 2;
    __shared__ int2 s_xy[GT_NV];
    __shared__ float s_iw[GT_NV];
// ... 123 lines not shown
        if (ms) {
            unsigned base = 0;
            if (lane == 0) base = atomicAdd(&s_nslow, (unsigned)__popcll(ms));
            base = (unsigned)__builtin_amdgcn_readfirstlane((int)base);
            if (kind == 2) s_q[GT_NC - 1 - (base + __popcll(ms & ((1ull << lane) - 1ull)))] = (unsigned short)id;
        }
        const unsigned long long mc = __ballot(kind == 3);
        if (mc) {
            unsigned base = 0;
            if (lane == 0) base = atomicAdd(&s_npark[2], (unsigned)__popcll(mc));
            base = (unsigned)__builtin_amdgcn_readfirstlane((int)base);
            if (kind == 3) s_park[base + __popcll(mc & ((1ull << lane) - 1ull))] = (unsigned short)id;
        }
    }
    __syncthreads();
    WGT(2);
    const int nfast = (int)s_nfast, nslow = (int)s_nslow;
    const unsigned ncell = s_npark[2];
#if defined(GRID_STOP_AFTER) && GRID_STOP_AFTER == 2
    if (nfast + nslow == 123456) vis[0] = s_q[threadIdx.x];
    return;
#endif
#ifdef ALP_RASTER_STATS
    {
        __shared__ int s_bb[4];
        __shared__ unsigned s_boxpix[3];
        if (threadIdx.x == 0) { s_bb[0] = INT_MAX; s_bb[1] = INT_MIN; s_bb[2] = INT_MAX; s_bb[3] = INT_MIN; s_boxpix[0] = s_boxpix[1] = s_boxpix[2] = 0; }
        __syncthreads();
        bool sentinel = false;
        for (int i = threadIdx.x; i < GT_NV; i += 256) {
            const int2 P = s_xy[i];
            if (P.x > NODATA) { atomicMin(&s_bb[0], P.x); atomicMax(&s_bb[1], P.x); atomicMin(&s_bb[2], P.y); atomicMax(&s_bb[3], P.y); }
            else if (P.x != BEHIND || true) sentinel |= (P.x == RANGE);
        }
        auto boxpix = [&](int id) {
            int lr, lc; cell_rc(id, lr, lc);
            const int ia = lr * GT_VW + lc;
            const int2 P0 = s_xy[ia], P1 = s_xy[ia + GT_VW], P2 = s_xy[ia + GT_VW + 1], P3 = s_xy[ia + 1];
            if (!(P0.x > NODATA && P1.x > NODATA && P2.x > NODATA && P3.x > NODATA)) return 0;
            const int minx = min(min(P0.x, P1.x), min(P2.x, P3.x)), maxx = max(max(P0.x, P1.x), max(P2.x, P3.x));
            const int miny = min(min(P0.y, P1.y), min(P2.y, P3.y)), maxy = max(max(P0.y, P1.y), max(P2.y, P3.y));
            const int i0 = max((minx + SUB / 2 - 1) >> 8, 0), i1 = min((maxx - SUB / 2) >> 8, v.w - 1);
            const int j0 = max((miny + SUB / 2 - 1) >> 8, 0), j1 = min((maxy - SUB / 2) >> 8, v.h - 1);
            return (i1 >= i0 && j1 >= j0) ? (i1 - i0 + 1) * (j1 - j0 + 1) : 0;
        };
        for (int e = threadIdx.x; e < nfast; e += 256) atomicAdd(&s_boxpix[0], (unsigned)boxpix(s_q[e]));
        for (int e = threadIdx.x; e < nslow; e += 256) atomicAdd(&s_boxpix[1], (unsigned)boxpix(s_q[GT_NC - 1 - e]));
        for (int e = threadIdx.x; e < (int)ncell; e += 256) atomicAdd(&s_boxpix[2], (unsigned)boxpix(s_park[e]));
        __syncthreads();
        if (threadIdx.x == 0) {
            const int i0 = max((s_bb[0] + SUB / 2 - 1) >> 8, 0), i1 = min((s_bb[1] - SUB / 2) >> 8, v.w - 1);
            const int j0 = max((s_bb[2] + SUB / 2 - 1) >> 8, 0), j1 = min((s_bb[3] - SUB / 2) >> 8, v.h - 1);
            const long long area = (i1 >= i0 && j1 >= j0) ? (long long)(((i1 - i0 + 8) & ~7)) * (j1 - j0 + 1) : 0;
            const int b = area <= 512 ? 0 : area <= 1024 ? 1 : area <= 2048 ? 2 : area <= 4096 ? 3 : area <= 8192 ? 4 : area <= 16384 ? 5 : area <= 65536 ? 6 : 7;
            RSTAT(24 + 8 * b + 0, 1);
            RSTAT(24 + 8 * b + 1, area);
            RSTAT(24 + 8 * b + 2, nfast);
            RSTAT(24 + 8 * b + 3, nslow);
            RSTAT(24 + 8 * b + 4, ncell);
            RSTAT(24 + 8 * b + 5, s_boxpix[0]);
            RSTAT(24 + 8 * b + 6, s_boxpix[1]);
            RSTAT(24 + 8 * b + 7, s_boxpix[2]);
        }
        __syncthreads();
    }
#endif
    if (threadIdx.x == 0) {
        RSTAT(10, 1);
        RSTAT(11, nfast);
        RSTAT(12, nslow);
        RSTAT(13, (nfast + 63) / 64);
        RSTAT(14, (nslow + 63) / 64);
    }
    int pI0 = 0, pJ0 = 0, pW = 0, pH = 0;
    bool use_patch = false;
    if (patch_cap && nfast >= PATCH_MIN_FAST) {
        const int x0 = min(min(s_wbb[0][0], s_wbb[1][0]), min(s_wbb[2][0], s_wbb[3][0]));
        const int x1 = max(max(s_wbb[0][1], s_wbb[1][1]), max(s_wbb[2][1], s_wbb[3][1]));
        const int y0 = min(min(s_wbb[0][2], s_wbb[1][2]), min(s_wbb[2][2], s_wbb[3][2]));
        const int y1 = max(max(s_wbb[0][3], s_wbb[1][3]), max(s_wbb[2][3], s_wbb[3][3]));
        const int i0 = max((x0 + SUB / 2 - 1) >> 8, 0), i1 = min((x1 - SUB / 2) >> 8, v.w - 1);
        const int j0 = max((y0 + SUB / 2 - 1) >> 8, 0), j1 = min((y1 - SUB / 2) >> 8, v.h - 1);
        if (i1 >= i0 && j1 >= j0) {
            pI0 = i0 & ~7;
            pJ0 = j0;
            pW = (i1 - pI0 + 8) & ~7;
            pH = j1 - j0 + 1;
            use_patch = mul24(pW, pH) <= patch_cap;
        }
    }
    const int patch_n = use_patch ? mul24(pW, pH) : 0;
    if (use_patch) {
        for (int k = threadIdx.x; k < patch_n; k += 256) s_patch[k] = 0ull;
        __syncthreads();
    }
    auto fast_cells = [&](auto to_patch) {
    constexpr bool PATCH = decltype(to_patch)::value;
    auto sink = [&](int i, int j, unsigned long long key) {
        if constexpr (PATCH)
            __hip_atomic_fetch_max(&s_patch[mul24(j - pJ0, pW) + (i - pI0)], key, __ATOMIC_RELAXED, __HIP_MEMORY_SCOPE_WORKGROUP);
        else
            vis_max(vis, v, i, j, key);
    };
#pragma unroll 1
    for (int e = threadIdx.x; e < nfast; e += 256) {
        const int id = s_q[e];
        int lr, lc;
        cell_rc(id, lr, lc);
        const int ia = lr * GT_VW + lc, ib = ia + GT_VW, ic = ib + 1, idd = ia + 1;
        const int2 a = s_xy[ia], b = s_xy[ib], cc = s_xy[ic], d = s_xy[idd];
        const unsigned cell = (unsigned)(r0 + lr) * (unsigned)(gw - 1) + (unsigned)(c0 + lc);
        const int minx = min(min(a.x, b.x), min(cc.x, d.x)), maxx = max(max(a.x, b.x), max(cc.x, d.x));
        const int miny = min(min(a.y, b.y), min(cc.y, d.y)), maxy = max(max(a.y, b.y), max(cc.y, d.y));
        const int ci0 = max((minx + SUB / 2 - 1) >> 8, 0), ci1 = min((maxx - SUB / 2) >> 8, v.w - 1);
        const int cj0 = max((miny + SUB / 2 - 1) >> 8, 0), cj1 = min((maxy - SUB / 2) >> 8, v.h - 1);
        const int px = ci0 * SUB + SUB / 2, py = cj0 * SUB + SUB / 2;
        const int pax = px - a.x, pay = py - a.y, pbx = px - b.x, pby = py - b.y;
        const int pcx = px - cc.x, pcy = py - cc.y, pdx = px - d.x, pdy = py - d.y;
        int ex[6] = {cc.x - b.x, a.x - cc.x, b.x - a.x, d.x - cc.x, a.x - d.x, 0};
        int ey[6] = {cc.y - b.y, a.y - cc.y, b.y - a.y, d.y - cc.y, a.y - d.y, 0};
        ex[5] = -ex[1];
        ey[5] = -ey[1];
        int bs[6], row[6];
        row[0] = mul24(ex[0], pby) - mul24(ey[0], pbx);
        row[1] = mul24(ex[1], pcy) - mul24(ey[1], pcx);
        row[2] = mul24(ex[2], pay) - mul24(ey[2], pax);
        row[3] = mul24(ex[3], pcy) - mul24(ey[3], pcx);
        row[4] = mul24(ex[4], pdy) - mul24(ey[4], pdx);
        row[5] = -row[1];
        const int area0 = row[0] + row[1] + row[2], area1 = row[3] + row[4] + row[5];
#pragma unroll
        for (int k = 0; k < 6; ++k) {
            bs[k] = 1 + (((ey[k] << 12) - ex[k]) >> 31);
            row[k] -= bs[k];
        }
        const float iwa = s_iw[ia], iwb = s_iw[ib], iwc = s_iw[ic], iwd = s_iw[idd];
        const float inv0 = exact_rcp_unchecked((float)area0), inv1 = exact_rcp_unchecked((float)area1);
        const unsigned long long lo0 = 0xFFFFFFFFu - 2u * cell, lo1 = lo0 - 1u;
        for (int j = cj0; j <= cj1; ++j) {
            int u[6];
#pragma unroll
            for (int k = 0; k < 6; ++k) u[k] = row[k];
            for (int i = ci0; i <= ci1; ++i) {
                if ((u[0] | u[1] | u[2]) >= 0) {
                    const float q = __builtin_fmaf((float)(u[2] + bs[2]), iwc,
                                                   __builtin_fmaf((float)(u[1] + bs[1]), iwb,
                                                                  (float)(u[0] + bs[0]) * iwa)) * inv0;
                    sink(i, j, ((unsigned long long)__float_as_uint(q) << 32) | lo0);
                }
                if ((u[3] | u[4] | u[5]) >= 0) {
                    const float q = __builtin_fmaf((float)(u[5] + bs[5]), iwd,
                                                   __builtin_fmaf((float)(u[4] + bs[4]), iwc,
                                                                  (float)(u[3] + bs[3]) * iwa)) * inv1;
                    sink(i, j, ((unsigned long long)__float_as_uint(q) << 32) | lo1);
                }
#pragma unroll
                for (int k = 0; k < 6; ++k) u[k] -= ey[k] * SUB;
            }
#pragma unroll
            for (int k = 0; k < 6; ++k) row[k] += ex[k] * SUB;
        }
    }
    };
    if (use_patch) {
        fast_cells(std::true_type{});
        __syncthreads();
        const int step_rows = 256 / pW, step_cols = 256 - step_rows * pW;
        int row = (int)threadIdx.x / pW, col = (int)threadIdx.x - row * pW;
        for (int k = threadIdx.x; k < patch_n; k += 256) {
            const unsigned long long key = s_patch[k];
            if (key) vis_max(vis, v, pI0 + col, pJ0 + row, key);
            row += step_rows;
            col += step_cols;
            if (col >= pW) { col -= pW; ++row; }
        }
    } else {
        fast_cells(std::false_type{});
    }
#if defined(GRID_STOP_AFTER) && GRID_STOP_AFTER == 3
    return;
#endif
#ifdef ALP_WG_TIMING
    __syncthreads();
#endif
    WGT(3);
#pragma unroll 1
    for (int e0 = (int)(threadIdx.x & ~63u); e0 < nslow; e0 += 256) {
        const int e = e0 + lane;
        const bool work = e < nslow;
        const int id = work ? (int)s_q[GT_NC - 1 - e] : 0;
        int lr, lc;
        cell_rc(id, lr, lc);
        const int ia = lr * GT_VW + lc, ib = ia + GT_VW, ic = ib + 1, idd = ia + 1;
        const int2 P0 = s_xy[ia], P1 = s_xy[ib], P2 = s_xy[ic], P3 = s_xy[idd];
        const unsigned cell = (unsigned)(r0 + lr) * (unsigned)(gw - 1) + (unsigned)(c0 + lc);
#pragma unroll
        for (int half = 0; half < 2; ++half) {
            const int k1 = half ? ic : ib, k2 = half ? idd : ic;
            const int2 A = P0, B = half ? P2 : P1, C = half ? P3 : P2;
            const unsigned t = 2u * cell + (unsigned)half;
            Deferred park;
            int code = EMIT_DONE;
            if (work) {
                if (A.x > NODATA && B.x > NODATA && C.x > NODATA) {
                    const int X[3] = {A.x, B.x, C.x}, Y[3] = {A.y, B.y, C.y};
                    code = emit_small(v, X, Y, s_iw, ia, k1, k2, t, vis, &park, true, COOP_MIN_W, COOP_MIN_PIX, true);
                } else if (A.x != NODATA && B.x != NODATA && C.x != NODATA &&
                           !(A.x == BEHIND && B.x == BEHIND && C.x == BEHIND)) {
                    code = EMIT_GENERAL;
                }
                if (code == EMIT_GENERAL) {
                    const unsigned slot = atomicAdd(gcount, 1u);
                    if (slot < gcap) gqueue[slot] = t;
                }
            }
            const unsigned long long ms = __ballot(code == EMIT_PARKED_SMALL), ml = __ballot(code == EMIT_PARKED);
            if (ms) {
                unsigned base = 0;
                if (lane == 0) base = atomicAdd(&s_npark[0], (unsigned)__popcll(ms));
                base = (unsigned)__builtin_amdgcn_readfirstlane((int)base);
                if (code == EMIT_PARKED_SMALL) s_park[ncell + base + __popcll(ms & ((1ull << lane) - 1ull))] = (unsigned short)(2 * id + half);
            }
            if (ml) {
                unsigned base = 0;
                if (lane == 0) base = atomicAdd(&s_npark[1], (unsigned)__popcll(ml));
                base = (unsigned)__builtin_amdgcn_readfirstlane((int)base);
                if (code == EMIT_PARKED) s_park[2 * GT_NC - 1 - (base + __popcll(ml & ((1ull << lane) - 1ull)))] = (unsigned short)(2 * id + half);
            }
        }
    }
    __syncthreads();
    const unsigned np_small = s_npark[0], np_large = s_npark[1];
    if (np_small + np_large + ncell == 0) {
        WGT(4);
        return;
    }
    if (threadIdx.x < 3) {
        const unsigned cnt = threadIdx.x == 0 ? np_small : (threadIdx.x == 1 ? np_large : ncell);
        s_park_base[threadIdx.x] = cnt ? atomicAdd(park_counts + threadIdx.x, cnt) : 0u;
    }
    __syncthreads();
    for (unsigned e = threadIdx.x; e < ncell; e += 256) {
        const int id = (int)s_park[e];
        int lr, lc;
        cell_rc(id, lr, lc);
        const int ia = lr * GT_VW + lc, ib = ia + GT_VW, ic = ib + 1, idd = ia + 1;
        const int2 A = s_xy[ia], B = s_xy[ib], C = s_xy[ic], D = s_xy[idd];
#ifdef ALP_RASTER_STATS
        {
            const int minx = min(min(A.x, B.x), min(C.x, D.x)), maxx = max(max(A.x, B.x), max(C.x, D.x));
            const int miny = min(min(A.y, B.y), min(C.y, D.y)), maxy = max(max(A.y, B.y), max(C.y, D.y));
            const int bw = min((maxx - SUB / 2) >> 8, v.w - 1) - max((minx + SUB / 2 - 1) >> 8, 0) + 1;
            const int bh = min((maxy - SUB / 2) >> 8, v.h - 1) - max((miny + SUB / 2 - 1) >> 8, 0) + 1;
            RSTAT(19, bh <= 2 ? 1 : 0);
            RSTAT(20, bh <= 4 ? 1 : 0);
            RSTAT(21, bw <= 4 ? 1 : 0);
            RSTAT(22, bw * bh);
// ... 37 lines not shown
```

### alproj_amd/csrc/raster_large.h

```cpp
#pragma once

template <bool IMPLICIT>
__global__ __launch_bounds__(256) void raster_large_kernel(const float *__restrict__ vert,
                                                           const int *__restrict__ ind, long long gw, View v,
                                                           unsigned long long *__restrict__ vis,
                                                           const WorkItem *__restrict__ queue,
                                                           const unsigned *__restrict__ qcount, unsigned qcap) {
    const unsigned count = min(*qcount, qcap);
    const int lane = threadIdx.x & 63;
    const unsigned wave = (blockIdx.x * blockDim.x + threadIdx.x) >> 6;
    const unsigned nwaves = (gridDim.x * blockDim.x) >> 6;
    for (unsigned it = wave; it < count; it += nwaves) {
        const WorkItem wi = queue[it];
        float q[3][3];
        load_view_tri<IMPLICIT>(v, vert, ind, gw, (long long)wi.tri, q);
        if (wi.sub == 0xFFFF) {
            raster_big(v, q, wi.tri, vis, lane);
            continue;
        }
        float xw[4], yw[4], iw[4];
        bool big;
        const int ntri = clip_project(v, q, xw, yw, iw, big);
        const int f = wi.sub;
        if (f >= ntri) continue;
        const float x3[3] = {xw[0], xw[f + 1], xw[f + 2]}, y3[3] = {yw[0], yw[f + 1], yw[f + 2]},
                    i3[3] = {iw[0], iw[f + 1], iw[f + 2]};
        const TriSetup s = setup_tri(v, x3, y3, i3);
        if (!s.valid) continue;
        const int i = wi.tx * TILE + lane;
        int ja = wi.ty * TILE, jb = ja + TILE - 1;
        ja = ja < s.j0 ? s.j0 : ja;
        jb = jb > s.j1 ? s.j1 : jb;
        if (i < s.i0 || i > s.i1) continue;
        for (int j = ja; j <= jb; ++j) {
            const unsigned long long key = pixel_key(s, i, j, wi.tri);
            if (key) vis_max(vis, v, i, j, key);
        }
    }
}
```

### alproj_amd/csrc/raster_parked.h

```cpp
#pragma once

__device__ __forceinline__ void park_append(bool take, const Deferred &d, Deferred *__restrict__ queue,
                                            unsigned *__restrict__ count, unsigned cap) {
    const unsigned long long m = __ballot(take);
    if (!m) return;
    const int lane = (int)(threadIdx.x & 63), leader = __ffsll((long long)m) - 1;
    unsigned base = 0;
#ifdef PARK_NOATOMIC
    base = (blockIdx.x * 64u) % (cap - 64u);
#else
    if (lane == leader) base = atomicAdd(count, (unsigned)__popcll(m));
    base = (unsigned)__builtin_amdgcn_readlane((int)base, leader);
#endif
    const unsigned slot = base + (unsigned)__popcll(m & ((1ull << lane) - 1ull));
    if (take && slot < cap) queue[slot] = d;
}

__device__ __forceinline__ void raster_coop_body(const View &v, unsigned long long *__restrict__ vis,
                                                 const Deferred *__restrict__ queue,
                                                 const unsigned *__restrict__ count, unsigned cap) {
    const unsigned n = min(*count, cap);
    const int lane = (int)(threadIdx.x & 63);
    const unsigned chunk = (n + 7u) >> 3, xcd = blockIdx.x & 7u, lo = xcd * chunk, hi = min(lo + chunk, n);
    const unsigned wave = (unsigned)__builtin_amdgcn_readfirstlane((int)(((blockIdx.x >> 3) * blockDim.x + threadIdx.x) >> 6));
    const unsigned nwaves = ((gridDim.x >> 3) * blockDim.x) >> 6;
    if (lo + wave >= hi) return;
    Deferred nextd = queue[lo + wave];
    for (unsigned it = lo + wave; it < hi; it += nwaves) {
        const Deferred d = nextd;
        if (it + nwaves < hi) nextd = queue[it + nwaves];
        int X[3], Y[3];
        float iw3[3];
#pragma unroll
        for (int k = 0; k < 3; ++k) {
            X[k] = __builtin_amdgcn_readfirstlane(d.X[k]);
            Y[k] = __builtin_amdgcn_readfirstlane(d.Y[k]);
            iw3[k] = __int_as_float(__builtin_amdgcn_readfirstlane(__float_as_int(d.iw[k])));
        }
        coop_raster(v, X, Y, iw3, (unsigned)__builtin_amdgcn_readfirstlane((int)d.t), vis, lane);
    }
}

__device__ __forceinline__ void raster_coop4_body(const View &v, unsigned long long *__restrict__ vis,
                                                  const Deferred *__restrict__ queue,
                                                  const unsigned *__restrict__ count, unsigned cap) {
    const unsigned n = min(*count, cap);
    const unsigned chunk = (n + 7u) >> 3, xcd = blockIdx.x & 7u, lo = xcd * chunk, hi = min(lo + chunk, n);
    const unsigned group = ((blockIdx.x >> 3) * blockDim.x + threadIdx.x) >> 4, ngroups = ((gridDim.x >> 3) * blockDim.x) >> 4;
    const int lx = (int)(threadIdx.x & 3), ly = (int)((threadIdx.x >> 2) & 3);
    if (lo + group >= hi) return;
    Deferred nextd = queue[lo + group];
    for (unsigned it = lo + group; it < hi; it += ngroups) {
        const Deferred d = nextd;
        if (it + ngroups < hi) nextd = queue[it + ngroups];
        const int minx = min(d.X[0], min(d.X[1], d.X[2])), maxx = max(d.X[0], max(d.X[1], d.X[2]));
        const int miny = min(d.Y[0], min(d.Y[1], d.Y[2])), maxy = max(d.Y[0], max(d.Y[1], d.Y[2]));
        const int ci0 = max((minx + SUB / 2 - 1) >> 8, 0), ci1 = min((maxx - SUB / 2) >> 8, v.w - 1);
        const int cj0 = max((miny + SUB / 2 - 1) >> 8, 0), cj1 = min((maxy - SUB / 2) >> 8, v.h - 1);
        const int area2 = mul24(d.X[1] - d.X[0], d.Y[2] - d.Y[0]) - mul24(d.X[2] - d.X[0], d.Y[1] - d.Y[0]);
        int dx[3], dy[3], bias[3];
#pragma unroll
        for (int k = 0; k < 3; ++k) {
            const int a = (k + 1) % 3, b = (k + 2) % 3;
            dx[k] = d.X[b] - d.X[a];
            dy[k] = d.Y[b] - d.Y[a];
            bias[k] = (dy[k] < 0 || (dy[k] == 0 && dx[k] > 0)) ? 0 : 1;
        }
        const float inv_area = exact_rcp_unchecked((float)area2);
        const unsigned long long lo = (unsigned long long)(0xFFFFFFFFu - d.t);
        for (int by = cj0; by <= cj1; by += 4)
            for (int bx = ci0 & ~3; bx <= ci1; bx += 4) {
                const int i = bx + lx, j = by + ly;
                if (i < ci0 || i > ci1 || j > cj1) continue;
                const int px = i * SUB + SUB / 2, py = j * SUB + SUB / 2;
                const int w0 = mul24(dx[0], py - d.Y[1]) - mul24(dy[0], px - d.X[1]) - bias[0];
                const int w1 = mul24(dx[1], py - d.Y[2]) - mul24(dy[1], px - d.X[2]) - bias[1];
                const int w2 = mul24(dx[2], py - d.Y[0]) - mul24(dy[2], px - d.X[0]) - bias[2];
                if ((w0 | w1 | w2) >= 0) {
                    const float q = __builtin_fmaf((float)(w2 + bias[2]), d.iw[2],
                                                   __builtin_fmaf((float)(w1 + bias[1]), d.iw[1],
                                                                  (float)(w0 + bias[0]) * d.iw[0])) * inv_area;
                    vis_max(vis, v, i, j, ((unsigned long long)__float_as_uint(q) << 32) | lo);
                }
            }
    }
}

__device__ __forceinline__ void raster_cell_body(const View &v, unsigned long long *__restrict__ vis,
                                                 const ParkedCell *__restrict__ queue,
                                                 const unsigned *__restrict__ count, unsigned cap) {
    const unsigned n = min(*count, cap);
    const int lane = (int)(threadIdx.x & 63), lx = lane & 7, ly = lane >> 3;
    const unsigned wave = (unsigned)__builtin_amdgcn_readfirstlane((int)((blockIdx.x * blockDim.x + threadIdx.x) >> 6));
    const unsigned nwaves = (gridDim.x * blockDim.x) >> 6;
    for (unsigned it = wave; it < n; it += nwaves) {
        const ParkedCell *e = queue + it;
        const int ax = e->X[0], bx_ = e->X[1], cx = e->X[2], dx_ = e->X[3];
        const int ay = e->Y[0], by_ = e->Y[1], cy = e->Y[2], dy_ = e->Y[3];
        const float iwa = e->iw[0], iwb = e->iw[1], iwc = e->iw[2], iwd = e->iw[3];
        const unsigned cell = e->cell;
        const int minx = min(min(ax, bx_), min(cx, dx_)), maxx = max(max(ax, bx_), max(cx, dx_));
        const int miny = min(min(ay, by_), min(cy, dy_)), maxy = max(max(ay, by_), max(cy, dy_));
        const int ci0 = max((minx + SUB / 2 - 1) >> 8, 0), ci1 = min((maxx - SUB / 2) >> 8, v.w - 1);
        const int cj0 = max((miny + SUB / 2 - 1) >> 8, 0), cj1 = min((maxy - SUB / 2) >> 8, v.h - 1);
        const int ex0 = cx - bx_, ex1 = ax - cx, ex2 = bx_ - ax, ex3 = dx_ - cx, ex4 = ax - dx_, ex5 = -ex1;
        const int ey0 = cy - by_, ey1 = ay - cy, ey2 = by_ - ay, ey3 = dy_ - cy, ey4 = ay - dy_, ey5 = -ey1;
        const int bs0 = 1 + (((ey0 << 12) - ex0) >> 31), bs1 = 1 + (((ey1 << 12) - ex1) >> 31), bs2 = 1 + (((ey2 << 12) - ex2) >> 31);
        const int bs3 = 1 + (((ey3 << 12) - ex3) >> 31), bs4 = 1 + (((ey4 << 12) - ex4) >> 31), bs5 = 1 + (((ey5 << 12) - ex5) >> 31);
        const int area0 = ex1 * (by_ - cy) - ey1 * (bx_ - cx) + ex2 * (by_ - ay) - ey2 * (bx_ - ax);
        const int area1 = ex4 * (cy - dy_) - ey4 * (cx - dx_);
        const float inv0 = exact_rcp_unchecked((float)area0), inv1 = exact_rcp_unchecked((float)area1);
        const unsigned long long lo0 = 0xFFFFFFFFu - 2u * cell, lo1 = lo0 - 1u;
        const int i = ci0 + lx, j = cj0 + ly;
        if (i > ci1 || j > cj1) continue;
        const int px = i * SUB + SUB / 2, py = j * SUB + SUB / 2;
        const int r0 = mul24(ex0, py - by_) - mul24(ey0, px - bx_);
        const int r1 = mul24(ex1, py - cy) - mul24(ey1, px - cx);
        const int r2 = mul24(ex2, py - ay) - mul24(ey2, px - ax);
        const int r3 = mul24(ex3, py - cy) - mul24(ey3, px - cx);
        const int r4 = mul24(ex4, py - dy_) - mul24(ey4, px - dx_);
        const int r5 = -r1;
        unsigned long long key = 0;
        if (((r0 - bs0) | (r1 - bs1) | (r2 - bs2)) >= 0) {
            const float q = __builtin_fmaf((float)r2, iwc, __builtin_fmaf((float)r1, iwb, (float)r0 * iwa)) * inv0;
            key = ((unsigned long long)__float_as_uint(q) << 32) | lo0;
        }
        if (((r3 - bs3) | (r4 - bs4) | (r5 - bs5)) >= 0) {
            const float q = __builtin_fmaf((float)r5, iwd, __builtin_fmaf((float)r4, iwc, (float)r3 * iwa)) * inv1;
            const unsigned long long k1 = ((unsigned long long)__float_as_uint(q) << 32) | lo1;
            key = k1 > key ? k1 : key;
        }
        if (key) vis_max(vis, v, i, j, key);
    }
}

__global__ __launch_bounds__(256) void raster_parked_kernel(View v, unsigned long long *__restrict__ vis,
                                                            const Deferred *__restrict__ small_q, const Deferred *__restrict__ large_q,
                                                            const ParkedCell *__restrict__ cell_q,
                                                            const unsigned *__restrict__ counts, unsigned cap_small,
                                                            unsigned cap_large, unsigned cap_cell) {
#ifndef PARKED_SKIP_CELLS
    raster_cell_body(v, vis, cell_q, counts + 2, cap_cell);
#endif
#ifndef PARKED_SKIP_COOP
    raster_coop_body(v, vis, large_q, counts + 1, cap_large);
#endif
#ifndef PARKED_SKIP_COOP4
    raster_coop4_body(v, vis, small_q, counts + 0, cap_small);
#endif
}
```

### alproj_amd/csrc/raster_plan.h

```cpp
#pragma once

#ifndef GT_W_LOG2
#define GT_W_LOG2 6
#endif
#ifndef GT_H_LOG2
#define GT_H_LOG2 4
#endif
constexpr int GT_W = 1 << GT_W_LOG2, GT_H = 1 << GT_H_LOG2, GT_VW = GT_W + 1, GT_VH = GT_H + 1, GT_NV = GT_VW * GT_VH,
              GT_NC = GT_W * GT_H;
static_assert(GT_NC % 256 == 0 && GT_NC <= 65536, "tile size");

constexpr int GT_DIV_SHIFT = 18;
constexpr int GT_DIV_MAGIC = ((1 << GT_DIV_SHIFT) + GT_VW - 1) / GT_VW;
constexpr bool gt_div_ok() {
    for (int i = 0; i < GT_NV; ++i)
        if (((i * GT_DIV_MAGIC) >> GT_DIV_SHIFT) != i / GT_VW) return false;
    return (long long)GT_NV * GT_DIV_MAGIC < (1ll << 31) && GT_DIV_MAGIC < (1 << 23);
}
static_assert(gt_div_ok(), "magic division");

__global__ __launch_bounds__(256) void tile_bounds_kernel(const float *__restrict__ vert, int gh, int gw, int tiles_x,
                                                          float *__restrict__ bounds) {
    __shared__ float s_min[4][3], s_max[4][3];
    const int tile_r = blockIdx.x / tiles_x, tile_c = blockIdx.x - tile_r * tiles_x;
// ... 142 lines not shown
        if (cull.enabled) {
            const float *tb = tile_bounds + 6ull * t;
            const float d0 = tb[0] - cull.cam[0], d1 = tb[1] - cull.cam[1], d2 = tb[2] - cull.cam[2];
            const float e0 = tb[3], e1 = tb[4], e2 = tb[5];
            const float a0 = fabsf(d0) + e0, a1 = fabsf(d1) + e1, a2 = fabsf(d2) + e2;
            const float g0 = fabsf(tb[0]) + fabsf(cull.cam[0]), g1 = fabsf(tb[1]) + fabsf(cull.cam[1]), g2 = fabsf(tb[2]) + fabsf(cull.cam[2]);
            bool outside = false;
            float vz_min = 0.0f;
#pragma unroll
            for (int k = 0; k < 5; ++k) {
                const float sd = cull.n[k][0] * d0 + cull.n[k][1] * d1 + cull.n[k][2] * d2;
                const float rr = cull.an[k][0] * e0 + cull.an[k][1] * e1 + cull.an[k][2] * e2;
                const float mg = 1e-5f * (cull.am[k][0] * a0 + cull.am[k][1] * a1 + cull.am[k][2] * a2) +
                                 4e-7f * (cull.am[k][0] * g0 + cull.am[k][1] * g1 + cull.am[k][2] * g2);
                if (k < 4) outside = outside || (sd - rr > mg);
                else {
                    outside = outside || (sd + rr < 1.0f - mg - 1e-5f);
                    vz_min = sd - rr - mg;
                }
            }
            if (outside) kind = 0;
            else if (cull.occlusion) {
                const float cell = fmaxf(2.0f * e0 / (float)GT_W, 2.0f * e2 / (float)GT_H);
                kind = (vz_min >= 2.0f && vz_min >= cull.near_limit * cell) ? 2 : 1;
                int px0, px1, py0, py1;
                float zmin;
                if (kind == 2 && far_tile_rect(tb, cull, px0, px1, py0, py1, zmin) && px0 <= px1 && py0 <= py1) {
                    reg[0] = 65535u - (unsigned)px0;
                    reg[1] = (unsigned)px1 + 1u;
                    reg[2] = 65535u - (unsigned)py0;
                    reg[3] = (unsigned)py1 + 1u;
                }
            }
        }
    }
    if (__ballot(reg[1] != 0u)) {
#pragma unroll
        for (int k = 0; k < 4; ++k) {
            const unsigned m = wave_max_to_lane63(reg[k]);
            if ((threadIdx.x & 63) == 63) atomicMax(&s_region[k], m);
        }
    }
    list_append(kind == 1, t, near_list, counts + 0);
    list_append(kind == 2, t, far_list, counts + 1);
    if (threadIdx.x < 4 && s_region[threadIdx.x]) atomicMax(region + threadIdx.x, s_region[threadIdx.x]);
}

#ifndef HIZ_SPAN
#define HIZ_SPAN 8
#endif
constexpr int HIZ_LEVELS = 4;

struct HizDims { int w[HIZ_LEVELS], h[HIZ_LEVELS]; long long off[HIZ_LEVELS]; };

static HizDims hiz_dims(int w, int h) {
    HizDims d;
    long long off = 0;
    for (int l = 0; l < HIZ_LEVELS; ++l) {
        const int b = 8 << l;
        d.w[l] = (w + b - 1) / b;
        d.h[l] = (h + b - 1) / b;
        d.off[l] = off;
        off += (long long)d.w[l] * d.h[l];
    }
    return d;
}
static long long hiz_total(int w, int h) {
    const HizDims d = hiz_dims(w, h);
    return d.off[HIZ_LEVELS - 1] + (long long)d.w[HIZ_LEVELS - 1] * d.h[HIZ_LEVELS - 1];
}

__global__ __launch_bounds__(256) void hiz_build_kernel(const unsigned long long *__restrict__ vis, int w, int h, HizDims dm,
                                                        unsigned *__restrict__ hiz, const unsigned *__restrict__ region) {
    __shared__ unsigned s_min[64 + 16 + 4 + 1];
    const int rx = blockIdx.x * 64, ry = blockIdx.y * 64;
    {
        const unsigned r0 = region[0], r1 = region[1], r2 = region[2], r3 = region[3];
        if (r1 == 0u || r3 == 0u) return;
        const int X0 = (int)(65535u - r0) & ~63, X1 = (int)(r1 - 1u) | 63, Y0 = (int)(65535u - r2) & ~63, Y1 = (int)(r3 - 1u) | 63;
        if (rx + 63 < X0 || rx > X1 || ry + 63 < Y0 || ry > Y1) return;
    }
    if (threadIdx.x < 85) s_min[threadIdx.x] = 0x7F800000u;
    __syncthreads();
    const int col = threadIdx.x & 63;
#pragma unroll 4
    for (int k = 0; k < 16; ++k) {
        const int row = (threadIdx.x >> 6) + 4 * k;
        const int x = rx + col, y = ry + row;
        if (x < w && y < h) {
            const unsigned q = (unsigned)(vis[(size_t)y * w + x] >> 32);
            atomicMin(&s_min[(row >> 3) * 8 + (col >> 3)], q);
        }
    }
    __syncthreads();
    if (threadIdx.x < 16) {
        const int bx = threadIdx.x & 3, by = threadIdx.x >> 2;
        unsigned m = 0x7F800000u;
        for (int j = 0; j < 2; ++j)
            for (int i = 0; i < 2; ++i) m = min(m, s_min[(2 * by + j) * 8 + 2 * bx + i]);
        s_min[64 + threadIdx.x] = m;
    }
    __syncthreads();
    if (threadIdx.x < 4) {
        const int bx = threadIdx.x & 1, by = threadIdx.x >> 1;
        unsigned m = 0x7F800000u;
        for (int j = 0; j < 2; ++j)
            for (int i = 0; i < 2; ++i) m = min(m, s_min[64 + (2 * by + j) * 4 + 2 * bx + i]);
        s_min[80 + threadIdx.x] = m;
    }
    __syncthreads();
    if (threadIdx.x == 0) s_min[84] = min(min(s_min[80], s_min[81]), min(s_min[82], s_min[83]));
    __syncthreads();
    if (threadIdx.x < 64) {
        const int tx = blockIdx.x * 8 + (threadIdx.x & 7), ty = blockIdx.y * 8 + (threadIdx.x >> 3);
        if (tx < dm.w[0] && ty < dm.h[0]) hiz[dm.off[0] + (long long)ty * dm.w[0] + tx] = s_min[threadIdx.x];
    } else if (threadIdx.x < 80) {
        const int k = threadIdx.x - 64, tx = blockIdx.x * 4 + (k & 3), ty = blockIdx.y * 4 + (k >> 2);
        if (tx < dm.w[1] && ty < dm.h[1]) hiz[dm.off[1] + (long long)ty * dm.w[1] + tx] = s_min[threadIdx.x];
    } else if (threadIdx.x < 84) {
        const int k = threadIdx.x - 80, tx = blockIdx.x * 2 + (k & 1), ty = blockIdx.y * 2 + (k >> 1);
        if (tx < dm.w[2] && ty < dm.h[2]) hiz[dm.off[2] + (long long)ty * dm.w[2] + tx] = s_min[threadIdx.x];
    } else if (threadIdx.x == 84) {
        hiz[dm.off[3] + (long long)blockIdx.y * dm.w[3] + blockIdx.x] = s_min[84];
    }
}

__global__ __launch_bounds__(256) void tile_occlusion_kernel(const float *__restrict__ tile_bounds, TileCull cull,
                                                             const unsigned *__restrict__ far_list,
                                                             const unsigned *__restrict__ counts, HizDims dm,
                                                             const unsigned *__restrict__ hiz, unsigned *__restrict__ out_list,
                                                             unsigned *__restrict__ out_count) {
    const unsigned i = blockIdx.x * blockDim.x + threadIdx.x;
    const unsigned n = counts[1];
    bool keep = false;
    unsigned t = 0;
    if (i < n) {
        t = far_list[i];
        keep = true;
        int px0, px1, py0, py1;
        float zmin;
        if (far_tile_rect(tile_bounds + 6ull * t, cull, px0, px1, py0, py1, zmin)) {
            if (px0 > px1 || py0 > py1) {
                keep = false;
            } else {
                const float *tb = tile_bounds + 6ull * t;
                const float zabs = 4e-7f * (fabsf(cull.R[2][0]) * (fabsf(tb[0]) + fabsf(cull.cam[0])) + fabsf(cull.R[2][1]) * (fabsf(tb[1]) + fabsf(cull.cam[1])) +
                                            fabsf(cull.R[2][2]) * (fabsf(tb[2]) + fabsf(cull.cam[2])));
                const float qmax = (1.0f / (zmin - zabs)) * 1.00002f;
                int L = 0;
                while (L < 3 && (((px1 >> (3 + L)) - (px0 >> (3 + L))) >= HIZ_SPAN || ((py1 >> (3 + L)) - (py0 >> (3 + L))) >= HIZ_SPAN)) ++L;
                const int tx0 = px0 >> (3 + L), tx1 = px1 >> (3 + L), ty0 = py0 >> (3 + L), ty1 = py1 >> (3 + L);
                if (tx1 - tx0 < 8 && ty1 - ty0 < 8) {
                    unsigned m = 0x7F800000u;
                    for (int ty = ty0; ty <= ty1; ++ty)
                        for (int tx = tx0; tx <= tx1; ++tx)
                            m = min(m, hiz[dm.off[L] + (long long)ty * dm.w[L] + tx]);
                    keep = !(qmax < __uint_as_float(m));
                }
            }
        }
    }
    list_append(keep, t, out_list, out_count);
}
```

### alproj_amd/csrc/raster_post.h

```cpp
#pragma once

constexpr int COMPACT_CHUNK = 4096;

__global__ __launch_bounds__(256) void image_u8_kernel(const float *__restrict__ img, long long npix, float scale, int reverse,
                                                       unsigned char *__restrict__ out) {
    const long long stride = (long long)gridDim.x * blockDim.x;
    for (long long i = (long long)blockIdx.x * blockDim.x + threadIdx.x; i < npix; i += stride) {
        unsigned char b[3];
#pragma unroll
        for (int c = 0; c < 3; ++c) {
            const float x = img[3 * i + c] * scale;
            const int q = (x >= -2147483648.0f && x < 2147483648.0f) ? (int)x : (int)0x80000000;
            b[c] = (unsigned char)(q & 0xFF);
        }
        out[3 * i + 0] = reverse ? b[2] : b[0];
        out[3 * i + 1] = b[1];
        out[3 * i + 2] = reverse ? b[0] : b[2];
    }
}

__global__ __launch_bounds__(256) void gather_pixels_kernel(const float *__restrict__ image, int w, int h,
                                                            const int *__restrict__ u, const int *__restrict__ v,
                                                            long long n, double o0, double o1, double o2,
                                                            double *__restrict__ xyz) {
// ... 178 lines not shown
    else if (b == a + gw + 1 && c == a + 1) type = 1;
    else return -1;
    if (a < 0) return -1;
    const unsigned row = (unsigned)a / (unsigned)gw, col = (unsigned)a - row * (unsigned)gw;
    if ((long long)row >= gh - 1 || (long long)col >= gw - 1) return -1;
    return 2 * ((long long)row * (gw - 1) + col) + type;
}

__global__ __launch_bounds__(256) void subgrid_mark_kernel(const int *__restrict__ ind, long long n_tri, long long gw, long long gh,
                                                           unsigned *__restrict__ present, unsigned char *__restrict__ mark,
                                                           unsigned *__restrict__ mismatch) {
    const long long stride = (long long)gridDim.x * blockDim.x;
    const long long rounds = (n_tri + stride - 1) / stride;
    const int lane = (int)(threadIdx.x & 63);
    bool bad = false;
    for (long long k = 0; k < rounds; ++k) {
        const long long t = k * stride + (long long)blockIdx.x * blockDim.x + threadIdx.x;
        const bool in = t < n_tri;
        const long long id = in ? subgrid_id(ind, t, gw, gh) : -1;
        long long prev = __shfl_up(id, 1);
        if (lane == 0) prev = (in && t > 0) ? subgrid_id(ind, t - 1, gw, gh) : -1;
        const bool ok = in && id >= 0 && !(t > 0 && prev >= id);
        bad |= in && !ok;
        const long long word = ok ? (id >> 5) : (-1 - lane);
        const long long wprev = __shfl_up(word, 1);
        const bool head = lane == 0 || wprev != word;
        const unsigned long long heads = __ballot(head);
        const int run = __popcll(heads & (~0ull >> (63 - lane)));
        unsigned bits = ok ? (1u << (id & 31)) : 0u;
#pragma unroll
        for (int j = 0; j < 6; ++j) {
            const unsigned b2 = __shfl_down(bits, 1 << j);
            const int r2 = __shfl_down(run, 1 << j);
            if ((lane + (1 << j) < 64) && r2 == run) bits |= b2;
        }
        if (ok) {
            if (head) atomicOr(&present[word], bits);
            mark[ind[3 * t]] = 1;
            mark[ind[3 * t + 1]] = 1;
            mark[ind[3 * t + 2]] = 1;
        }
    }
    if (bad) *mismatch = 1u;
}

__global__ __launch_bounds__(256) void subgrid_absent_kernel(long long n_grid_tri, long long gw, const unsigned *__restrict__ present,
                                                             const unsigned char *__restrict__ mark, unsigned *__restrict__ mismatch) {
    const long long stride = (long long)gridDim.x * blockDim.x;
    bool bad = false;
    for (long long id = (long long)blockIdx.x * blockDim.x + threadIdx.x; id < n_grid_tri; id += stride) {
        if (present[id >> 5] >> (id & 31) & 1u) continue;
        const Idx3 e = tri_vertices<true>(nullptr, gw, id);
        bad |= mark[e.a] && mark[e.b] && mark[e.c];
    }
    if (bad) *mismatch = 1u;
}

__global__ __launch_bounds__(256) void subgrid_blocksum_kernel(const unsigned *__restrict__ present, long long n_words,
                                                               unsigned *__restrict__ block_sums) {
    __shared__ unsigned s[4];
    const long long w = (long long)blockIdx.x * 256 + threadIdx.x;
    unsigned c = w < n_words ? (unsigned)__popc(present[w]) : 0u;
    for (int m = 32; m >= 1; m >>= 1) c += __shfl_xor(c, m, 64);
    if ((threadIdx.x & 63) == 0) s[threadIdx.x >> 6] = c;
    __syncthreads();
    if (threadIdx.x == 0) block_sums[blockIdx.x] = s[0] + s[1] + s[2] + s[3];
}

__global__ __launch_bounds__(256) void subgrid_rank_kernel(const unsigned *__restrict__ present, long long n_words,
                                                           const unsigned *__restrict__ block_offsets, unsigned *__restrict__ rank) {
    __shared__ unsigned s[256];
    const long long w = (long long)blockIdx.x * 256 + threadIdx.x;
    s[threadIdx.x] = w < n_words ? (unsigned)__popc(present[w]) : 0u;
    __syncthreads();
    for (int d = 1; d < 256; d <<= 1) {
        const unsigned t = threadIdx.x >= (unsigned)d ? s[threadIdx.x - d] : 0u;
        __syncthreads();
        s[threadIdx.x] += t;
        __syncthreads();
    }
    if (w < n_words) rank[w] = block_offsets[blockIdx.x] + (threadIdx.x ? s[threadIdx.x - 1] : 0u);
}

__global__ __launch_bounds__(256) void vis_translate_kernel(const unsigned long long *__restrict__ vis, long long npix,
                                                            const unsigned *__restrict__ present, const unsigned *__restrict__ rank,
                                                            unsigned long long *__restrict__ out) {
    const long long p = (long long)blockIdx.x * blockDim.x + threadIdx.x;
    if (p >= npix) return;
    unsigned long long key = vis[p];
    if (key) {
        const unsigned id = 0xFFFFFFFFu - (unsigned)(key & 0xFFFFFFFFull);
        const unsigned pos = rank[id >> 5] + (unsigned)__popc(present[id >> 5] & ((1u << (id & 31)) - 1u));
        key = (key & 0xFFFFFFFF00000000ull) | (unsigned long long)(0xFFFFFFFFu - pos);
    }
    out[p] = key;
}

__global__ __launch_bounds__(256) void mask_and_kernel(const unsigned char *__restrict__ derived, const unsigned char *__restrict__ user,
                                                       long long n, unsigned char *__restrict__ out) {
    const long long i = (long long)blockIdx.x * blockDim.x + threadIdx.x;
    if (i < n) out[i] = derived[i] && (!user || user[i]);
}

__global__ __launch_bounds__(256) void cast_f64_f32_kernel(const double *__restrict__ src, long long count, long long dst_off,
                                                           float *__restrict__ dst) {
    const long long stride = (long long)gridDim.x * blockDim.x;
    for (long long i = (long long)blockIdx.x * blockDim.x + threadIdx.x; i < count; i += stride) dst[dst_off + i] = (float)src[i];
}

__global__ __launch_bounds__(256) void check_index_range_kernel(const int *__restrict__ ind, long long count, long long n_vert,
                                                                unsigned *__restrict__ bad) {
    const long long stride = (long long)gridDim.x * blockDim.x;
    unsigned mine = 0;
    for (long long i = (long long)blockIdx.x * blockDim.x + threadIdx.x; i < count; i += stride) {
        const int v = ind[i];
        mine += (v < 0 || v >= n_vert) ? 1u : 0u;
    }
    if (mine) atomicAdd(bad, mine);
}

__global__ __launch_bounds__(256) void narrow_indices_kernel(const long long *__restrict__ src, long long count,
                                                             long long dst_off, int *__restrict__ dst, long long n_vert,
                                                             unsigned *__restrict__ bad) {
    const long long stride = (long long)gridDim.x * blockDim.x;
    unsigned mine = 0;
    for (long long i = (long long)blockIdx.x * blockDim.x + threadIdx.x; i < count; i += stride) {
        const long long v = src[i];
        mine += (v < 0 || v >= n_vert) ? 1u : 0u;
        dst[dst_off + i] = (int)v;
    }
    if (mine) atomicAdd(bad, mine);
}
```

### alproj_amd/csrc/raster_resolve.h

```cpp
#pragma once

__device__ __forceinline__ bool remap_source(const RemapCoef &c, int w, int h, int x, int y, int &sx, int &sy,
                                             float *mapx = nullptr, float *mapy = nullptr) {
    const double x1 = (x - c.c0) / c.c0, y1 = (y - c.c1) / c.c1;
    const double r = __builtin_sqrt(x1 * x1 + y1 * y1), r2 = r * r, r4 = r2 * r2, r6 = r4 * r2;
    const double xd = x1 * (1 + c.k1 * r2 + c.k2 * r4 + c.k3 * r6) / (1 + c.k4 * r2 + c.k5 * r4 + c.k6 * r6) +
                      2 * c.p1 * x1 * y1 + c.p2 * (r2 * 2 * x1 * x1) + c.s1 * r2 + c.s2 * r4;
    const double yd = y1 * (1 + c.a1 + c.k1 * r2 + c.k2 * r4 + c.k3 * r6) / (1 + c.a2 + c.k4 * r2 + c.k5 * r4 + c.k6 * r6) +
                      2 * c.p1 * x1 * y1 + c.p2 * (r2 * 2 * y1 * y1) + c.s3 * r2 + c.s4 * r4;
    const float mx = (float)(xd * c.c0 + c.c0), my = (float)(yd * c.c1 + c.c1);
    if (mapx) { *mapx = mx; *mapy = my; }
    const double rx = __builtin_rint((double)mx), ry = __builtin_rint((double)my);
    if (!(rx >= 0 && rx < w && ry >= 0 && ry < h)) return false;
    sx = (int)rx;
    sy = (int)ry;
    return true;
}

__global__ __launch_bounds__(256) void distort_map_kernel(int w, int h, RemapCoef rc, float *__restrict__ map_x,
                                                          float *__restrict__ map_y) {
    const long long npix = (long long)w * h;
    const long long stride = (long long)gridDim.x * blockDim.x;
    for (long long p = (long long)blockIdx.x * blockDim.x + threadIdx.x; p < npix; p += stride) {
        const int y = (int)(p / w), x = (int)(p - (long long)y * w);
        int sx, sy;
        remap_source(rc, w, h, x, y, sx, sy, map_x + p, map_y + p);
    }
}

#ifndef RESOLVE_BLOCKS_PER_CU
#define RESOLVE_BLOCKS_PER_CU 64
#endif
template <bool IMPLICIT>
__global__ __launch_bounds__(256) void resolve_kernel(const float *__restrict__ vert, const float *__restrict__ value,
                                                      const int *__restrict__ ind, long long gw, View v,
                                                      RemapCoef rc, int identity_remap, double min_distance,
                                                      const unsigned long long *__restrict__ vis,
                                                      float *__restrict__ out, const unsigned *__restrict__ frame_counts,
                                                      unsigned *__restrict__ host_counts) {
    if (host_counts && blockIdx.x == 0 && threadIdx.x < 2 * QC_STRIDE) host_counts[threadIdx.x] = frame_counts[threadIdx.x];
    const long long npix = (long long)v.w * v.h;
    const long long stride = (long long)gridDim.x * blockDim.x;
    for (long long p = (long long)blockIdx.x * blockDim.x + threadIdx.x; p < npix; p += stride) {
        const int y = (int)((unsigned)p / (unsigned)v.w), x = (int)((unsigned)p - (unsigned)y * (unsigned)v.w);
        float o[3] = {0.0f, 0.0f, 0.0f};
        int sx, sy;
        if (identity_remap ? (sx = x, sy = y, true) : remap_source(rc, v.w, v.h, x, y, sx, sy)) {
            const int j = v.h - 1 - sy;
            const unsigned long long key = vis[(size_t)j * v.w + sx];
            if (key) {
                const long long t = (long long)(0xFFFFFFFFu - (unsigned)(key & 0xFFFFFFFFull));
                const Idx3 id = tri_vertices<IMPLICIT>(ind, gw, t);
                const long long ids[3] = {id.a, id.b, id.c};
                double Q[3][3];
                float P[3][3];
#pragma unroll
                for (int k = 0; k < 3; ++k) {
                    const float *pp = vert + 3 * ids[k];
                    P[k][0] = pp[0];
                    P[k][1] = pp[1];
                    P[k][2] = pp[2];
                    const double d0 = (double)P[k][0] - v.camd[0], d1 = (double)P[k][1] - v.camd[1], d2 = (double)P[k][2] - v.camd[2];
#pragma unroll
                    for (int c = 0; c < 3; ++c) Q[k][c] = (v.Rd[c][0] * d0 + v.Rd[c][1] * d1) + v.Rd[c][2] * d2;
                }
                const double *A = Q[0], *B = Q[1], *C = Q[2];
                const double r[3] = {(((double)sx + 0.5) * v.kx - 1.0) * v.ifx,
                                     (((double)j + 0.5) * v.ky - 1.0) * v.ify, 1.0};
                const double e1[3] = {B[0] - A[0], B[1] - A[1], B[2] - A[2]}, e2[3] = {C[0] - A[0], C[1] - A[1], C[2] - A[2]};
                const double pv[3] = {r[1] * e2[2] - r[2] * e2[1], r[2] * e2[0] - r[0] * e2[2], r[0] * e2[1] - r[1] * e2[0]};
                const double det = e1[0] * pv[0] + e1[1] * pv[1] + e1[2] * pv[2];
                const double tv[3] = {-A[0], -A[1], -A[2]};
                const double inv_det = 1.0 / det;
                const double beta = (tv[0] * pv[0] + tv[1] * pv[1] + tv[2] * pv[2]) * inv_det;
                const double qv[3] = {tv[1] * e1[2] - tv[2] * e1[1], tv[2] * e1[0] - tv[0] * e1[2], tv[0] * e1[1] - tv[1] * e1[0]};
                const double gamma = (r[0] * qv[0] + r[1] * qv[1] + r[2] * qv[2]) * inv_det;
                const double alpha = 1.0 - beta - gamma;
                bool masked = false;
                if (min_distance > 0) {
                    const double dA = __builtin_sqrt(A[0] * A[0] + A[1] * A[1] + A[2] * A[2]);
                    const double dB = __builtin_sqrt(B[0] * B[0] + B[1] * B[1] + B[2] * B[2]);
                    const double dC = __builtin_sqrt(C[0] * C[0] + C[1] * C[1] + C[2] * C[2]);
                    masked = alpha * dA + beta * dB + gamma * dC < min_distance;
                }
                if (!masked) {
                    if (value) {
#pragma unroll
                        for (int k = 0; k < 3; ++k) {
                            const float *pv_ = value + 3 * ids[k];
                            P[k][0] = pv_[0];
                            P[k][1] = pv_[1];
                            P[k][2] = pv_[2];
                        }
                    }
#pragma unroll
                    for (int c = 0; c < 3; ++c) o[c] = (float)(alpha * P[0][c] + beta * P[1][c] + gamma * P[2][c]);
                }
            }
        }
        out[p * 3 + 0] = o[0];
        out[p * 3 + 1] = o[1];
        out[p * 3 + 2] = o[2];
    }
}

__global__ __launch_bounds__(256) void distort_image_kernel(const float *__restrict__ img, int w, int h, int c,
                                                            RemapCoef rc, float *__restrict__ out) {
    const long long npix = (long long)w * h;
    const long long stride = (long long)gridDim.x * blockDim.x;
    for (long long p = (long long)blockIdx.x * blockDim.x + threadIdx.x; p < npix; p += stride) {
        const int y = (int)(p / w), x = (int)(p - (long long)y * w);
        int sx, sy;
        const bool ok = remap_source(rc, w, h, x, y, sx, sy);
        for (int k = 0; k < c; ++k) out[p * c + k] = ok ? img[((long long)sy * w + sx) * c + k] : 0.0f;
    }
}
```

Measured before the change: 503.6.

## Store visibility buffer in 4x2 pixel blocks instead of row-major

Introduces a VisLayout template that stores the 64-bit visibility keys in small 2D blocks (4x2 pixels by default) so each 64-byte line covers a compact screen region. All writers (raster kernels, patch flush, parked and large-triangle paths), readers (resolve, hi-z build, translate) and lane-to-pixel mappings are rewritten to use the blocked index, and the resolve kernel now walks 64x4 tiles. The aim is better cache-line locality for atomic max writes from small triangles, at the cost of extra index arithmetic, padded buffers, and a translate pass when fetching visibility.

```diff
diff --git a/alproj_amd/csrc/alp_raster.hip b/alproj_amd/csrc/alp_raster.hip
--- a/alproj_amd/csrc/alp_raster.hip
+++ b/alproj_amd/csrc/alp_raster.hip
@@ -203,12 +203,14 @@
 
 namespace {
 
+size_t vis_words(int w, int h) { return (size_t)VisL::words((uint32_t)w, (uint32_t)h); }
+
 int ensure_frame(alp_mesh *m, int w, int h) {
     if (m->w == w && m->h == h && m->vis) return ALP_OK;
     m->w = m->h = 0;
     m->vis_current = false;
     reset_all(m->vis, m->image);
-    if (int rc = reserve_all({(size_t)w * h * sizeof(unsigned long long) + QC_TOTAL * sizeof(unsigned),
+    if (int rc = reserve_all({vis_words(w, h) * sizeof(unsigned long long) + QC_TOTAL * sizeof(unsigned),
                               (size_t)w * h * 3 * sizeof(float)}, m->vis, m->image))
         return rc;
     m->hiz.reset();
@@ -218,7 +220,7 @@
     return ALP_OK;
 }
 
-unsigned *frame_counters(const alp_mesh *m, const View &v) { return (unsigned *)(m->vis + (size_t)v.w * v.h); }
+unsigned *frame_counters(const alp_mesh *m, const View &v) { return (unsigned *)(m->vis + vis_words(v.w, v.h)); }
 
 host::FramePlan frame_plan_of(const alp_mesh *m, const View &v) {
     return host::frame_plan(m->implicit, m->grid_h, m->grid_w, m->n_tri, v.w, v.h, ctx().cu_count, GT_W, GT_H, RASTER_BLOCKS_PER_CU,
@@ -339,7 +341,7 @@
     const host::FramePlan p = frame_plan_of(m, v);
     m->vis_current = false;
     if (!resolve_only)
-        ALP_HIP(hipMemsetAsync(m->vis, 0, (size_t)v.w * v.h * sizeof(unsigned long long) + QC_TOTAL * sizeof(unsigned), st));
+        ALP_HIP(hipMemsetAsync(m->vis, 0, vis_words(v.w, v.h) * sizeof(unsigned long long) + QC_TOTAL * sizeof(unsigned), st));
     if (m->n_tri > 0 && !resolve_only) {
         if (m->implicit)
             if (int e = ensure_grid_plan(m, p)) return e;
@@ -629,11 +631,11 @@
     if (!m->rendered) return fail(ALP_ESTATE, "alp_render_fetch_visibility: nothing rendered yet");
     if (int e = finish_frame(m)) return e;
     const unsigned long long *src = m->vis;
-    if (m->tri_present) {
-        const long long npix = (long long)m->w * m->h;
+    if (m->tri_present || !VisL::ROW_MAJOR) {
+        const long long npix = (long long)m->w * m->h, words = (long long)vis_words(m->w, m->h);
         unsigned long long *tr = nullptr;
         if (int rc = scratch_reserve((size_t)npix * sizeof(uint64_t), (void **)&tr)) return rc;
-        hipLaunchKernelGGL(vis_translate_kernel, dim3((unsigned)((npix + 255) / 256)), dim3(256), 0, ctx().stream, m->vis, npix,
+        hipLaunchKernelGGL(vis_translate_kernel, dim3((unsigned)((words + 255) / 256)), dim3(256), 0, ctx().stream, m->vis, m->w, m->h,
                            m->tri_present, m->tri_rank, tr);
         ALP_HIP(hipGetLastError());
         src = tr;
@@ -866,7 +868,7 @@
     m->unchecked = false;
     if (int e = ensure_frame(m, (int)w, (int)h)) return e;
     if (int e = upload_chunked(m->image, image, (size_t)h * w * 3 * sizeof(float))) return e;
-    ALP_HIP(hipMemsetAsync(m->vis, 0, (size_t)h * w * sizeof(unsigned long long), ctx().stream));
+    ALP_HIP(hipMemsetAsync(m->vis, 0, vis_words((int)w, (int)h) * sizeof(unsigned long long), ctx().stream));
     m->vis_current = false;
     m->rz_n = -1;
     m->rendered = true;
diff --git a/alproj_amd/csrc/alp_raster_internal.h b/alproj_amd/csrc/alp_raster_internal.h
--- a/alproj_amd/csrc/alp_raster_internal.h
+++ b/alproj_amd/csrc/alp_raster_internal.h
@@ -8,6 +8,7 @@
     float camf[3], caml[3];
     float fx, fy, sx, sy;
     int w, h;
+    int vis_pitch;
     double fxd, fyd;
     double kx, ky, ifx, ify;
     double Rd[3][3], camd[3];
diff --git a/alproj_amd/csrc/host/alp_host_selfcheck.cpp b/alproj_amd/csrc/host/alp_host_selfcheck.cpp
--- a/alproj_amd/csrc/host/alp_host_selfcheck.cpp
+++ b/alproj_amd/csrc/host/alp_host_selfcheck.cpp
@@ -472,6 +472,91 @@
             ok &= rd.div(k * w) == k && rd.div(k * w - 1) == k - 1;
         }
         if (!ok) CHECK(false, "RowDiv::div is not e / %u somewhere below 2^31", w);
+    }
+}
+
+template <int BW_LOG2>
+void check_vis_layout_of() {
+    using L = VisLayout<BW_LOG2>;
+    constexpr uint32_t HMAX = 300;
+    std::vector<uint32_t> seen;
+    for (uint32_t w = 1; w <= 300; ++w) {
+        const uint32_t pitch = L::pitch(w), wpad = L::ROW_MAJOR ? w : (w + L::BW - 1) / L::BW * L::BW;
+        bool ok = true;
+        seen.assign((size_t)L::words(w, HMAX), 0);
+        uint32_t top = 0, taken = 0;
+        for (uint32_t j = 0; j < HMAX; ++j) {
+            for (uint32_t i = 0; i < w; ++i) {
+                const uint32_t q = L::index(i, j, pitch);
+                ok &= q < seen.size();
+                if (!ok) break;
+                ok &= seen[q]++ == 0;
+                top = q > top ? q : top;
+                if (L::ROW_MAJOR) ok &= q == j * w + i;
+                uint32_t pi = ~0u, pj = ~0u;
+                L::pixel(q, pitch, &pi, &pj);
+                ok &= pi == i && pj == j;
+                if (!L::ROW_MAJOR && i + 1 < w) ok &= (L::index(i + 1, j, pitch) >> 3 == q >> 3) == ((i + 1) / L::BW == i / L::BW);
+                if (!L::ROW_MAJOR) ok &= (L::index(i, j + 1, pitch) >> 3 == q >> 3) == ((j + 1) / L::BH == j / L::BH);
+            }
+            if (!ok) break;
+            taken += w;
+            const uint32_t h = j + 1, hpad = (h + L::BH - 1) / L::BH * L::BH;
+            const uint64_t words = L::words(w, h);
+            ok &= words == (uint64_t)wpad * hpad && top < words && L::padded_h(h) == hpad;
+            uint32_t free_words = 0;
+            for (uint64_t q = words - (uint64_t)pitch; q < words; ++q) {
+                uint32_t pi = 0, pj = 0;
+                L::pixel((uint32_t)q, pitch, &pi, &pj);
+                const bool inside = pi < w && pj < h;
+                ok &= inside == (seen[q] != 0);
+                free_words += inside ? 0 : 1;
+            }
+            ok &= (uint64_t)taken + free_words + (uint64_t)(hpad - L::BH) * (wpad - w) == words;
+            if (!ok) { CHECK(false, "VisLayout<%d>: frame %u x %u", BW_LOG2, w, h); break; }
+        }
+        if (!ok) CHECK(false, "VisLayout<%d>: width %u", BW_LOG2, w);
+    }
+    const uint32_t W = 32768, H = 32768, pitch = L::pitch(W);
+    CHECK(pitch < (1u << 24) && L::words(W, H) <= (1ull << 31), "VisLayout<%d>: the largest frame leaves the 24-bit factors", BW_LOG2);
+    CHECK(L::index(W - 1, H - 1, pitch) == L::words(W, H) - 1 && L::index(0, 0, pitch) == 0, "VisLayout<%d>: corners of the largest frame", BW_LOG2);
+    uint32_t pi = 0, pj = 0;
+    L::pixel((uint32_t)(L::words(W, H) - 1), pitch, &pi, &pj);
+    CHECK(pi == W - 1 && pj == H - 1, "VisLayout<%d>: last word of the largest frame", BW_LOG2);
+}
+
+template <class L, int WX, int WY>
+void check_window_lane() {
+    constexpr int N = 1 << (WX + WY);
+    bool taken[N] = {false};
+    bool ok = true;
+    const uint32_t pitch = L::pitch(1u << WX);
+    for (int l = 0; l < N; ++l) {
+        int x = -1, y = -1;
+        L::template window_lane<WX, WY>(l, &x, &y);
+        ok &= x >= 0 && x < (1 << WX) && y >= 0 && y < (1 << WY) && !taken[(y << WX) + x];
+        if (!ok) break;
+        taken[(y << WX) + x] = true;
+        int x0, y0;
+        constexpr int G = L::ROW_MAJOR ? (WX < 3 ? 1 << WX : 8) : (N < 8 ? N : 8);
+        L::template window_lane<WX, WY>(l & ~(G - 1), &x0, &y0);
+        if (L::ROW_MAJOR) ok &= y == y0 && (x >> 3) == (x0 >> 3);
+        else if ((1 << WX) >= L::BW && (1 << WY) >= L::BH) ok &= L::index((uint32_t)x, (uint32_t)y, pitch) >> 3 == L::index((uint32_t)x0, (uint32_t)y0, pitch) >> 3;
+    }
+    CHECK(ok, "VisLayout<%d>::window_lane<%d, %d>", L::BW_L2, WX, WY);
+}
+
+void check_vis_layout() {
+    check_vis_layout_of<1>();
+    check_vis_layout_of<2>();
+    check_vis_layout_of<3>();
+    check_window_lane<VisLayout<1>, 3, 3>(); check_window_lane<VisLayout<2>, 3, 3>(); check_window_lane<VisLayout<3>, 3, 3>();
+    check_window_lane<VisLayout<1>, 2, 2>(); check_window_lane<VisLayout<2>, 2, 2>(); check_window_lane<VisLayout<3>, 2, 2>();
+    check_window_lane<VisLayout<1>, 4, 2>(); check_window_lane<VisLayout<2>, 5, 1>(); check_window_lane<VisLayout<3>, 6, 0>();
+    for (int l = 0; l < 64; ++l) {
+        int x, y;
+        VisLayout<3>::window_lane<3, 3>(l, &x, &y);
+        CHECK(x == (l & 7) && y == (l >> 3), "VisLayout<3>::window_lane<3, 3>(%d)", l);
     }
 }
 
@@ -1060,7 +1145,7 @@
                             {"convert", check_convert}, {"grid", check_grid},     {"selection", check_selection}, {"errors", check_errors},
                             {"plan", check_plan},       {"frame_plan", check_frame_plan}, {"row_div", check_row_div}, {"lm", check_lm},
                             {"buffer", check_buffer},   {"row_walk", check_row_walk}, {"match_plan", check_match_plan},
-                            {"epi_plan", check_epi_plan}};
+                            {"epi_plan", check_epi_plan}, {"vis_layout", check_vis_layout}};
     const bool concurrent = !(argc > 1 && !strcmp(argv[1], "--serial"));
     std::vector<std::thread> th;
     for (const Group &g : groups) {
diff --git a/alproj_amd/csrc/host/alp_plan.h b/alproj_amd/csrc/host/alp_plan.h
--- a/alproj_amd/csrc/host/alp_plan.h
+++ b/alproj_amd/csrc/host/alp_plan.h
@@ -36,6 +36,44 @@
             *col = e - r * rd.w;
             *row0 = r * rd.w;
         }
+    }
+};
+
+template <int BW_LOG2>
+struct VisLayout {
+    static_assert(BW_LOG2 >= 1 && BW_LOG2 <= 3, "blocks of 2 x 4, 4 x 2 or 8 x 1 pixels");
+    static constexpr int BW_L2 = BW_LOG2, BH_L2 = 3 - BW_LOG2, BW = 1 << BW_L2, BH = 1 << BH_L2;
+    static constexpr bool ROW_MAJOR = BH == 1;
+    ALP_HD static uint32_t pitch(uint32_t w) { return ROW_MAJOR ? w : ((w + BW - 1) >> BW_L2) << 3; }
+    ALP_HD static uint32_t padded_h(uint32_t h) { return (h + BH - 1) & ~(uint32_t)(BH - 1); }
+    ALP_HD static uint64_t words(uint32_t w, uint32_t h) { return (uint64_t)pitch(w) * (padded_h(h) >> BH_L2); }
+    ALP_HD static uint32_t mul(uint32_t a, uint32_t b) {
+#if defined(__HIP_DEVICE_COMPILE__)
+        return __umul24(a, b);
+#else
+        return a * b;
+#endif
+    }
+    ALP_HD static uint32_t index(uint32_t i, uint32_t j, uint32_t pitch) {
+        if (ROW_MAJOR) return mul(j, pitch) + i;
+        return mul(j >> BH_L2, pitch) + ((i >> BW_L2) << 3) + ((j & (BH - 1)) << BW_L2) + (i & (BW - 1));
+    }
+    ALP_HD static void pixel(uint32_t q, uint32_t pitch, uint32_t *i, uint32_t *j) {
+        const uint32_t br = q / pitch;
+        row_pixel(br, q - br * pitch, i, j);
+    }
+    ALP_HD static void row_pixel(uint32_t br, uint32_t r, uint32_t *i, uint32_t *j) {
+        if (ROW_MAJOR) { *i = r; *j = br; return; }
+        *i = ((r >> 3) << BW_L2) + (r & (BW - 1));
+        *j = (br << BH_L2) + ((r & 7) >> BW_L2);
+    }
+    template <int WX_L2, int WY_L2>
+    ALP_HD static void window_lane(int l, int *x, int *y) {
+        constexpr int XB = BW_L2 < WX_L2 ? BW_L2 : WX_L2, YB = BH_L2 < WY_L2 ? BH_L2 : WY_L2;
+        const int xin = l & ((1 << XB) - 1), yin = (l >> XB) & ((1 << YB) - 1);
+        const int xout = (l >> (XB + YB)) & ((1 << (WX_L2 - XB)) - 1), yout = l >> (WX_L2 + YB);
+        *x = xin | (xout << XB);
+        *y = yin | (yout << YB);
     }
 };
 
diff --git a/alproj_amd/csrc/raster_common.h b/alproj_amd/csrc/raster_common.h
--- a/alproj_amd/csrc/raster_common.h
+++ b/alproj_amd/csrc/raster_common.h
@@ -4,6 +4,10 @@
 constexpr float COORD_LIMIT = 4194304.0f;
 constexpr int SMALL_PIXELS = 32;
 constexpr int TILE = 64;
+#ifndef VIS_BW_LOG2
+#define VIS_BW_LOG2 2
+#endif
+using VisL = VisLayout<VIS_BW_LOG2>;
 
 static void make_view(const double *p, const double *offsets, View *v, RemapCoef *rc) {
     double x = p[0], y = p[1], z = p[2];
@@ -41,6 +45,7 @@
     v->fy = (float)v->fyd;
     v->w = (int)w;
     v->h = (int)h;
+    v->vis_pitch = (int)VisL::pitch((uint32_t)v->w);
     v->sx = 0.5f * (float)v->w;
     v->sy = 0.5f * (float)v->h;
     v->kx = 1.0 / (double)v->sx;
@@ -187,7 +192,7 @@
 }
 
 __device__ __forceinline__ void vis_max(unsigned long long *vis, const View &v, int i, int j, unsigned long long key) {
-    unsigned long long *dst = vis + (unsigned)(__umul24((unsigned)j, (unsigned)v.w) + (unsigned)i);
+    unsigned long long *dst = vis + VisL::index((unsigned)i, (unsigned)j, (unsigned)v.vis_pitch);
 #ifdef VIS_PLAIN_STORE
     __builtin_nontemporal_store(key, dst);
 #elif defined(VIS_NEVER)
@@ -241,10 +246,13 @@
     const double det = xh[0] * (yh[1] * wh[2] - yh[2] * wh[1]) - yh[0] * (xh[1] * wh[2] - xh[2] * wh[1]) +
                        wh[0] * (xh[1] * yh[2] - xh[2] * yh[1]);
     if (!(det > 0)) return;
-    const long long npix = (long long)v.w * v.h;
-    for (long long p = lane; p < npix; p += 64) {
+    const unsigned nword = (unsigned)VisL::words((unsigned)v.w, (unsigned)v.h);
+    for (unsigned p = lane; p < nword; p += 64) {
         {
-            const int j = (int)(p / v.w), i = (int)(p - (long long)j * v.w);
+            unsigned ui, uj;
+            VisL::pixel(p, (unsigned)v.vis_pitch, &ui, &uj);
+            const int i = (int)ui, j = (int)uj;
+            if (i >= v.w || j >= v.h) continue;
             const double px = i + 0.5, py = j + 0.5;
             double e[3];
             bool inside = true;
@@ -358,11 +366,12 @@
     }
     const float inv_area = exact_rcp_unchecked((float)area2);
     const unsigned long long lo = (unsigned long long)(0xFFFFFFFFu - t);
-    const int lx = lane & 7, ly = lane >> 3;
-    for (int by = cj0; by <= cj1; by += 8)
+    int lx, ly;
+    VisL::window_lane<3, 3>(lane, &lx, &ly);
+    for (int by = cj0 & ~(VisL::BH - 1); by <= cj1; by += 8)
         for (int bx = ci0 & ~7; bx <= ci1; bx += 8) {
             const int i = bx + lx, j = by + ly;
-            if (i < ci0 || i > ci1 || j > cj1) continue;
+            if (i < ci0 || i > ci1 || j < cj0 || j > cj1) continue;
             const int px = i * SUB + SUB / 2, py = j * SUB + SUB / 2;
             const int w0 = mul24(dx[0], py - ya[0]) - mul24(dy[0], px - xa[0]) - bias[0];
             const int w1 = mul24(dx[1], py - ya[1]) - mul24(dy[1], px - xa[1]) - bias[1];
diff --git a/alproj_amd/csrc/raster_dev.h b/alproj_amd/csrc/raster_dev.h
--- a/alproj_amd/csrc/raster_dev.h
+++ b/alproj_amd/csrc/raster_dev.h
@@ -10,7 +10,7 @@
 #endif
 #if defined(INLINE_LOG2) || defined(FAST_MAX) || defined(COOP_MIN_W) || defined(COOP_MIN_PIX) || defined(GT_W_LOG2) || defined(GT_H_LOG2) || \
     defined(HIZ_SPAN) || defined(GRID_WAVES_PER_EU) || defined(PATCH_MIN_FAST) || defined(PATCH_WORDS_NEAR) || defined(PATCH_WORDS_FAR) ||    \
-    defined(RASTER_BLOCKS_PER_CU) || defined(RESOLVE_BLOCKS_PER_CU)
+    defined(RASTER_BLOCKS_PER_CU) || defined(RESOLVE_BLOCKS_PER_CU) || defined(VIS_BW_LOG2)
 #define ALP_DEV_TUNABLES 1
 #ifndef ALP_DEV
 #error "tuning parameter overridden without -DALP_DEV"
diff --git a/alproj_amd/csrc/raster_grid.h b/alproj_amd/csrc/raster_grid.h
--- a/alproj_amd/csrc/raster_grid.h
+++ b/alproj_amd/csrc/raster_grid.h
@@ -229,14 +229,19 @@
         const int i0 = max((x0 + SUB / 2 - 1) >> 8, 0), i1 = min((x1 - SUB / 2) >> 8, v.w - 1);
         const int j0 = max((y0 + SUB / 2 - 1) >> 8, 0), j1 = min((y1 - SUB / 2) >> 8, v.h - 1);
         if (i1 >= i0 && j1 >= j0) {
-            pI0 = i0 & ~7;
-            pJ0 = j0;
-            pW = (i1 - pI0 + 8) & ~7;
-            pH = j1 - j0 + 1;
+            constexpr int XA = VisL::ROW_MAJOR ? 8 : VisL::BW;
+            pI0 = i0 & ~(XA - 1);
+            pJ0 = j0 & ~(VisL::BH - 1);
+            pW = (i1 - pI0 + XA) & ~(XA - 1);
+            pH = (j1 - pJ0 + VisL::BH) & ~(VisL::BH - 1);
             use_patch = mul24(pW, pH) <= patch_cap;
+#ifdef ALP_RASTER_STATS
+            if (threadIdx.x == 0) RSTAT(9, (mul24((i1 - (i0 & ~7) + 8) & ~7, j1 - j0 + 1) <= patch_cap && !use_patch) ? 1 : 0);
+#endif
         }
     }
     const int patch_n = use_patch ? mul24(pW, pH) : 0;
+    const unsigned patch_pitch = VisL::pitch((unsigned)pW);
     if (use_patch) {
         for (int k = threadIdx.x; k < patch_n; k += 256) s_patch[k] = 0ull;
         __syncthreads();
@@ -245,7 +250,8 @@
     constexpr bool PATCH = decltype(to_patch)::value;
     auto sink = [&](int i, int j, unsigned long long key) {
         if constexpr (PATCH)
-            __hip_atomic_fetch_max(&s_patch[mul24(j - pJ0, pW) + (i - pI0)], key, __ATOMIC_RELAXED, __HIP_MEMORY_SCOPE_WORKGROUP);
+            __hip_atomic_fetch_max(&s_patch[VisL::index((unsigned)(i - pI0), (unsigned)(j - pJ0), patch_pitch)], key, __ATOMIC_RELAXED,
+                                   __HIP_MEMORY_SCOPE_WORKGROUP);
         else
             vis_max(vis, v, i, j, key);
     };
@@ -312,14 +318,16 @@
     if (use_patch) {
         fast_cells(std::true_type{});
         __syncthreads();
-        const int step_rows = 256 / pW, step_cols = 256 - step_rows * pW;
-        int row = (int)threadIdx.x / pW, col = (int)threadIdx.x - row * pW;
+        const unsigned step_rows = 256u / patch_pitch, step_cols = 256u - step_rows * patch_pitch;
+        unsigned row = threadIdx.x / patch_pitch, col = threadIdx.x - row * patch_pitch;
         for (int k = threadIdx.x; k < patch_n; k += 256) {
             const unsigned long long key = s_patch[k];
-            if (key) vis_max(vis, v, pI0 + col, pJ0 + row, key);
+            unsigned pi, pj;
+            VisL::row_pixel(row, col, &pi, &pj);
+            if (key) vis_max(vis, v, pI0 + (int)pi, pJ0 + (int)pj, key);
             row += step_rows;
             col += step_cols;
-            if (col >= pW) { col -= pW; ++row; }
+            if (col >= patch_pitch) { col -= patch_pitch; ++row; }
         }
     } else {
         fast_cells(std::false_type{});
diff --git a/alproj_amd/csrc/raster_large.h b/alproj_amd/csrc/raster_large.h
--- a/alproj_amd/csrc/raster_large.h
+++ b/alproj_amd/csrc/raster_large.h
@@ -27,14 +27,18 @@
                     i3[3] = {iw[0], iw[f + 1], iw[f + 2]};
         const TriSetup s = setup_tri(v, x3, y3, i3);
         if (!s.valid) continue;
-        const int i = wi.tx * TILE + lane;
+        constexpr int SW_L2 = 6 - VisL::BH_L2, SW = 1 << SW_L2;
+        int lx, ly;
+        VisL::window_lane<SW_L2, VisL::BH_L2>(lane, &lx, &ly);
         int ja = wi.ty * TILE, jb = ja + TILE - 1;
         ja = ja < s.j0 ? s.j0 : ja;
         jb = jb > s.j1 ? s.j1 : jb;
-        if (i < s.i0 || i > s.i1) continue;
-        for (int j = ja; j <= jb; ++j) {
-            const unsigned long long key = pixel_key(s, i, j, wi.tri);
-            if (key) vis_max(vis, v, i, j, key);
-        }
+        for (int j0 = ja & ~(VisL::BH - 1); j0 <= jb; j0 += VisL::BH)
+            for (int i0 = wi.tx * TILE; i0 < wi.tx * TILE + TILE; i0 += SW) {
+                const int i = i0 + lx, j = j0 + ly;
+                if (i < s.i0 || i > s.i1 || j < ja || j > jb) continue;
+                const unsigned long long key = pixel_key(s, i, j, wi.tri);
+                if (key) vis_max(vis, v, i, j, key);
+            }
     }
 }
diff --git a/alproj_amd/csrc/raster_parked.h b/alproj_amd/csrc/raster_parked.h
--- a/alproj_amd/csrc/raster_parked.h
+++ b/alproj_amd/csrc/raster_parked.h
@@ -47,7 +47,9 @@
     const unsigned n = min(*count, cap);
     const unsigned chunk = (n + 7u) >> 3, xcd = blockIdx.x & 7u, lo = xcd * chunk, hi = min(lo + chunk, n);
     const unsigned group = ((blockIdx.x >> 3) * blockDim.x + threadIdx.x) >> 4, ngroups = ((gridDim.x >> 3) * blockDim.x) >> 4;
-    const int lx = (int)(threadIdx.x & 3), ly = (int)((threadIdx.x >> 2) & 3);
+    int lx, ly;
+    VisL::window_lane<2, 2>((int)(threadIdx.x & 15), &lx, &ly);
+    constexpr int YA = VisL::BH < 4 ? VisL::BH : 4;
     if (lo + group >= hi) return;
     Deferred nextd = queue[lo + group];
     for (unsigned it = lo + group; it < hi; it += ngroups) {
@@ -68,10 +70,10 @@
         }
         const float inv_area = exact_rcp_unchecked((float)area2);
         const unsigned long long lo = (unsigned long long)(0xFFFFFFFFu - d.t);
-        for (int by = cj0; by <= cj1; by += 4)
+        for (int by = cj0 & ~(YA - 1); by <= cj1; by += 4)
             for (int bx = ci0 & ~3; bx <= ci1; bx += 4) {
                 const int i = bx + lx, j = by + ly;
-                if (i < ci0 || i > ci1 || j > cj1) continue;
+                if (i < ci0 || i > ci1 || j < cj0 || j > cj1) continue;
                 const int px = i * SUB + SUB / 2, py = j * SUB + SUB / 2;
                 const int w0 = mul24(dx[0], py - d.Y[1]) - mul24(dy[0], px - d.X[1]) - bias[0];
                 const int w1 = mul24(dx[1], py - d.Y[2]) - mul24(dy[1], px - d.X[2]) - bias[1];
@@ -90,7 +92,9 @@
                                                  const ParkedCell *__restrict__ queue,
                                                  const unsigned *__restrict__ count, unsigned cap) {
     const unsigned n = min(*count, cap);
-    const int lane = (int)(threadIdx.x & 63), lx = lane & 7, ly = lane >> 3;
+    const int lane = (int)(threadIdx.x & 63);
+    int lx, ly;
+    VisL::window_lane<3, 3>(lane, &lx, &ly);
     const unsigned wave = (unsigned)__builtin_amdgcn_readfirstlane((int)((blockIdx.x * blockDim.x + threadIdx.x) >> 6));
     const unsigned nwaves = (gridDim.x * blockDim.x) >> 6;
     for (unsigned it = wave; it < n; it += nwaves) {
@@ -111,8 +115,13 @@
         const int area1 = ex4 * (cy - dy_) - ey4 * (cx - dx_);
         const float inv0 = exact_rcp_unchecked((float)area0), inv1 = exact_rcp_unchecked((float)area1);
         const unsigned long long lo0 = 0xFFFFFFFFu - 2u * cell, lo1 = lo0 - 1u;
-        const int i = ci0 + lx, j = cj0 + ly;
-        if (i > ci1 || j > cj1) continue;
+        int wi0 = ci0, wj0 = cj0;
+        if (!VisL::ROW_MAJOR) {
+            const int ai0 = ci0 & ~(VisL::BW - 1), aj0 = cj0 & ~(VisL::BH - 1);
+            if (ci1 - ai0 < 8 && cj1 - aj0 < 8) { wi0 = ai0; wj0 = aj0; }
+        }
+        const int i = wi0 + lx, j = wj0 + ly;
+        if (i < ci0 || i > ci1 || j < cj0 || j > cj1) continue;
         const int px = i * SUB + SUB / 2, py = j * SUB + SUB / 2;
         const int r0 = mul24(ex0, py - by_) - mul24(ey0, px - bx_);
         const int r1 = mul24(ex1, py - cy) - mul24(ey1, px - cx);
diff --git a/alproj_amd/csrc/raster_plan.h b/alproj_amd/csrc/raster_plan.h
--- a/alproj_amd/csrc/raster_plan.h
+++ b/alproj_amd/csrc/raster_plan.h
@@ -248,13 +248,14 @@
     }
     if (threadIdx.x < 85) s_min[threadIdx.x] = 0x7F800000u;
     __syncthreads();
-    const int col = threadIdx.x & 63;
+    const unsigned pitch = (unsigned)VisL::pitch((unsigned)w);
 #pragma unroll 4
     for (int k = 0; k < 16; ++k) {
-        const int row = (threadIdx.x >> 6) + 4 * k;
-        const int x = rx + col, y = ry + row;
+        unsigned col, row;
+        VisL::pixel(threadIdx.x + 256u * k, VisL::pitch(64u), &col, &row);
+        const int x = rx + (int)col, y = ry + (int)row;
         if (x < w && y < h) {
-            const unsigned q = (unsigned)(vis[(size_t)y * w + x] >> 32);
+            const unsigned q = (unsigned)(vis[VisL::index((unsigned)x, (unsigned)y, pitch)] >> 32);
             atomicMin(&s_min[(row >> 3) * 8 + (col >> 3)], q);
         }
     }
diff --git a/alproj_amd/csrc/raster_post.h b/alproj_amd/csrc/raster_post.h
--- a/alproj_amd/csrc/raster_post.h
+++ b/alproj_amd/csrc/raster_post.h
@@ -284,13 +284,17 @@
     if (w < n_words) rank[w] = block_offsets[blockIdx.x] + (threadIdx.x ? s[threadIdx.x - 1] : 0u);
 }
 
-__global__ __launch_bounds__(256) void vis_translate_kernel(const unsigned long long *__restrict__ vis, long long npix,
+__global__ __launch_bounds__(256) void vis_translate_kernel(const unsigned long long *__restrict__ vis, int w, int h,
                                                             const unsigned *__restrict__ present, const unsigned *__restrict__ rank,
                                                             unsigned long long *__restrict__ out) {
-    const long long p = (long long)blockIdx.x * blockDim.x + threadIdx.x;
-    if (p >= npix) return;
-    unsigned long long key = vis[p];
-    if (key) {
+    const long long q = (long long)blockIdx.x * blockDim.x + threadIdx.x;
+    if (q >= (long long)VisL::words((unsigned)w, (unsigned)h)) return;
+    unsigned i, j;
+    VisL::pixel((unsigned)q, VisL::pitch((unsigned)w), &i, &j);
+    if (i >= (unsigned)w || j >= (unsigned)h) return;
+    const long long p = (long long)j * w + i;
+    unsigned long long key = vis[q];
+    if (key && present) {
         const unsigned id = 0xFFFFFFFFu - (unsigned)(key & 0xFFFFFFFFull);
         const unsigned pos = rank[id >> 5] + (unsigned)__popc(present[id >> 5] & ((1u << (id & 31)) - 1u));
         key = (key & 0xFFFFFFFF00000000ull) | (unsigned long long)(0xFFFFFFFFu - pos);
diff --git a/alproj_amd/csrc/raster_resolve.h b/alproj_amd/csrc/raster_resolve.h
--- a/alproj_amd/csrc/raster_resolve.h
+++ b/alproj_amd/csrc/raster_resolve.h
@@ -39,15 +39,13 @@
                                                       float *__restrict__ out, const unsigned *__restrict__ frame_counts,
                                                       unsigned *__restrict__ host_counts) {
     if (host_counts && blockIdx.x == 0 && threadIdx.x < 2 * QC_STRIDE) host_counts[threadIdx.x] = frame_counts[threadIdx.x];
-    const long long npix = (long long)v.w * v.h;
-    const long long stride = (long long)gridDim.x * blockDim.x;
-    for (long long p = (long long)blockIdx.x * blockDim.x + threadIdx.x; p < npix; p += stride) {
-        const int y = (int)((unsigned)p / (unsigned)v.w), x = (int)((unsigned)p - (unsigned)y * (unsigned)v.w);
+    const unsigned vis_pitch = (unsigned)v.vis_pitch;
+    auto shade = [&](long long p, int x, int y) {
         float o[3] = {0.0f, 0.0f, 0.0f};
         int sx, sy;
         if (identity_remap ? (sx = x, sy = y, true) : remap_source(rc, v.w, v.h, x, y, sx, sy)) {
             const int j = v.h - 1 - sy;
-            const unsigned long long key = vis[(size_t)j * v.w + sx];
+            const unsigned long long key = vis[VisL::index((unsigned)sx, (unsigned)j, vis_pitch)];
             if (key) {
                 const long long t = (long long)(0xFFFFFFFFu - (unsigned)(key & 0xFFFFFFFFull));
                 const Idx3 id = tri_vertices<IMPLICIT>(ind, gw, t);
@@ -101,6 +99,22 @@
         out[p * 3 + 0] = o[0];
         out[p * 3 + 1] = o[1];
         out[p * 3 + 2] = o[2];
+    };
+    if constexpr (VisL::ROW_MAJOR) {
+        const long long npix = (long long)v.w * v.h;
+        const long long stride = (long long)gridDim.x * blockDim.x;
+        for (long long p = (long long)blockIdx.x * blockDim.x + threadIdx.x; p < npix; p += stride) {
+            const int y = (int)((unsigned)p / (unsigned)v.w), x = (int)((unsigned)p - (unsigned)y * (unsigned)v.w);
+            shade(p, x, y);
+        }
+    } else {
+        const unsigned tiles_x = ((unsigned)v.w + 63u) >> 6, tiles = tiles_x * (((unsigned)v.h + 3u) >> 2);
+        const int lx = (int)(threadIdx.x & 63), ly = (int)(threadIdx.x >> 6);
+        for (unsigned t = blockIdx.x; t < tiles; t += gridDim.x) {
+            const unsigned ty = t / tiles_x, tx = t - ty * tiles_x;
+            const int x = (int)(tx << 6) + lx, y = v.h - 1 - ((int)(ty << 2) + ly);
+            if (x < v.w && y >= 0) shade((long long)y * v.w + x, x, y);
+        }
     }
 }
 
```

New measurement: 504.3, median of 2. About the same (+0.1%).
